# gogojjh/M-LOAM

Hardware: NVIDIA B200
Metric: scan_to_map_lidar_frames_per_sec (higher is better)
Workload: dtype f32/f64

## Files before the change

### m-loam_b200/csrc/api.cu

```cuda
#include <cstdio>
#include <cstdlib>
#include <cstring>
#include <new>

#include "ctx.h"
#include "host_util.h"

using namespace mloam;

namespace mloam {

ProfScope::ProfScope(Ctx *ctx, const char *nm) : c(ctx), name(nm) {
  if (!c->prof_on) return;
  auto get = [&]() {
    cudaEvent_t e;
    if (!c->evt_pool.empty()) {
      e = c->evt_pool.back();
      c->evt_pool.pop_back();
    } else {
      cudaEventCreate(&e);
    }
    return e;
  };
  a = get();
  b = get();
  cudaEventRecord(a, c->stream);
}
ProfScope::~ProfScope() {
  if (!a) return;
  cudaEventRecord(b, c->stream);
  c->pending.push_back(Ctx::PendingEvt{name, a, b});
}
void prof_collect(Ctx *c) {
  for (auto &p : c->pending) {
    float ms = 0.f;
    if (cudaEventSynchronize(p.b) == cudaSuccess && cudaEventElapsedTime(&ms, p.a, p.b) == cudaSuccess) {
      ProfSlot &s = c->prof[p.name];
      s.ms += ms;
      s.launches += 1;
    }
    c->evt_pool.push_back(p.a);
    c->evt_pool.push_back(p.b);
  }
  c->pending.clear();
}

}

extern "C" {

const char *mloam_version(void) { return "mloam_b200 0.1 (sm_100a)"; }

void mloam_default_params(mloam_params_t *p) {
  memset(p, 0, sizeof(*p));
  p->n_scans = 64;
  p->distance_sq_threshold = 25.0f;
  p->nearby_scan = 2.5f;
  p->min_match_sq_dis = 1.0f;
  p->min_plane_dis = 0.2f;
  p->n_neigh = 5;
  p->check_fov = 0;
  p->point_plane_factor = 1;
  p->point_edge_factor = 1;
  p->huber_a = 0.1;
  p->eig_thre = 100.0;
  p->cov_trace = 0.0075;
  p->max_outer = 2;
  p->max_inner = 30;
  p->map_cell = 0.0f;
  p->corner_leaf = 0.2f;
  p->surf_leaf = 0.4f;
  p->gf_method = 0, p->gf_ratio = 1.0f, p->gf_seed = 0;
}

int mloam_ctx_create(int device, const mloam_params_t *params, mloam_ctx_t **out) {
  if (!out) return MLOAM_E_INVALID;
  *out = nullptr;
  int ndev = 0;
  if (cudaGetDeviceCount(&ndev) != cudaSuccess || ndev <= 0 || device < 0 || device >= ndev) return MLOAM_E_NO_DEVICE;
  cudaDeviceProp prop;
  if (cudaGetDeviceProperties(&prop, device) != cudaSuccess) return MLOAM_E_NO_DEVICE;
  if (prop.major != 10) {
    fprintf(stderr, "mloam_b200: device %d is sm_%d%d; this library carries sm_100a code only\n", device, prop.major,
            prop.minor);
    return MLOAM_E_NO_DEVICE;
  }
  if (cudaSetDevice(device) != cudaSuccess) return MLOAM_E_NO_DEVICE;
  mloam_ctx *h = new (std::nothrow) mloam_ctx();
  if (!h) return MLOAM_E_INVALID;
  Ctx *c = &h->c;
  c->device = device;
  c->sm_count = prop.multiProcessorCount;
  if (params) c->params = *params;
  else mloam_default_params(&c->params);
  if (cudaStreamCreateWithFlags(&c->stream, cudaStreamNonBlocking) != cudaSuccess ||
      cudaStreamCreateWithFlags(&c->stream2, cudaStreamNonBlocking) != cudaSuccess ||
      cudaEventCreateWithFlags(&c->ev_fork, cudaEventDisableTiming) != cudaSuccess ||
      cudaEventCreateWithFlags(&c->ev_join, cudaEventDisableTiming) != cudaSuccess ||
      cudaEventCreateWithFlags(&c->ev_maps, cudaEventDisableTiming) != cudaSuccess ||
      cudaStreamCreateWithFlags(&c->stream3, cudaStreamNonBlocking) != cudaSuccess ||
      cudaEventCreateWithFlags(&c->ev_fork3, cudaEventDisableTiming) != cudaSuccess ||
      cudaEventCreateWithFlags(&c->ev_join3, cudaEventDisableTiming) != cudaSuccess ||
      cudaStreamCreateWithFlags(&c->stream4, cudaStreamNonBlocking) != cudaSuccess ||
      cudaStreamCreateWithFlags(&c->stream5, cudaStreamNonBlocking) != cudaSuccess ||
      cudaEventCreateWithFlags(&c->ev_fork4, cudaEventDisableTiming) != cudaSuccess ||
      cudaEventCreateWithFlags(&c->ev_join4, cudaEventDisableTiming) != cudaSuccess ||
      cudaEventCreateWithFlags(&c->ev_fork5, cudaEventDisableTiming) != cudaSuccess ||
      cudaEventCreateWithFlags(&c->ev_join5, cudaEventDisableTiming) != cudaSuccess ||
      cudaEventCreateWithFlags(&c->ev_next, cudaEventDisableTiming) != cudaSuccess ||
      cudaMallocHost(&c->pinned, kPinnedBytes) != cudaSuccess || c->lm_state.reserve(sizeof(LMState) + 64) != cudaSuccess ||
      c->scratch[7].reserve(4096) != cudaSuccess) {
    delete h;
    return MLOAM_E_CUDA;
  }
  c->pinned_cap = kPinnedBytes;
  memset(c->pinned, 0, kPinnedBytes);
  cudaMemset(c->scratch[7].p, 0, 4096);
  if (const char *e = getenv("MLOAM_DISABLE_GRAPHS")) c->use_graphs = (e[0] == '0' || e[0] == '\0') ? 1 : 0;
  if (const char *e = getenv("MLOAM_KNN_TRACE")) c->knn_trace_on = e[0] == '1';
  if (const char *e = getenv("MLOAM_KNN_MB")) {
    const int v = atoi(e);
    if (v >= 2 && v <= 4) c->knn_min_blocks = v;
  }
  if (const char *e = getenv("MLOAM_KNN_TMA_MIN")) c->knn_tma_min = (unsigned)strtoul(e, nullptr, 10);
  if (const char *e = getenv("MLOAM_LOOKAHEAD")) c->use_lookahead = (e[0] == '0') ? 0 : 1;
  if (const char *e = getenv("MLOAM_STAMP")) c->stamp_on = e[0] == '1';
  if (const char *e = getenv("MLOAM_FUSE_ITER")) c->fuse_iter = (e[0] == '0') ? 0 : 1;
  if (const char *e = getenv("MLOAM_DISABLE_SEEDS")) c->use_seeds = (e[0] == '0' || e[0] == '\0') ? 1 : 0;
  *out = h;
  return MLOAM_OK;
}

void mloam_ctx_destroy(mloam_ctx_t *h) {
  if (!h) return;
  Ctx *c = &h->c;
  cudaSetDevice(c->device);
  cudaStreamSynchronize(c->stream);
  mloam_comm_destroy(h);
  for (auto &g : c->graphs)
    if (g.exec) cudaGraphExecDestroy(g.exec);
  c->graphs.clear();
  prof_collect(c);
  for (auto e : c->evt_pool) cudaEventDestroy(e);
  for (auto &m : c->maps) {
    m.sorted.release(), m.orig.release(), m.cells.release(), m.rank_of.release(), m.tile_sums.release(), m.hdr.release();
  }
  for (int i = 0; i < 4; i++) c->scan_pts[i].release(), c->feat_valid[i].release(), c->feat_coeff[i].release(), c->feat_nn[i].release(), c->knn_pos[i].release(), c->knn_changed[i].release(), c->knn_anchor[i].release(), c->knn_heavy[i].release();
  for (int i = 0; i < 2; i++) c->gf_work[i].release();
  c->knn_heavy_list.release(), c->knn_trace.release();
  c->partials.release(), c->lm_state.release();
  for (auto &s : c->scratch) s.release();
  c->frame_main.release(), c->frame_alt.release(), c->next_in.release(), c->stamps.release();
  if (c->pinned) cudaFreeHost(c->pinned);
  if (c->own_stream && c->stream) cudaStreamDestroy(c->stream);
  if (c->stream2) cudaStreamSynchronize(c->stream2), cudaStreamDestroy(c->stream2);
  if (c->ev_fork) cudaEventDestroy(c->ev_fork);
  if (c->ev_join) cudaEventDestroy(c->ev_join);
  if (c->ev_maps) cudaEventDestroy(c->ev_maps);
  if (c->stream3) cudaStreamSynchronize(c->stream3), cudaStreamDestroy(c->stream3);
  if (c->ev_fork3) cudaEventDestroy(c->ev_fork3);
  if (c->ev_join3) cudaEventDestroy(c->ev_join3);
  if (c->stream4) cudaStreamSynchronize(c->stream4), cudaStreamDestroy(c->stream4);
  if (c->stream5) cudaStreamSynchronize(c->stream5), cudaStreamDestroy(c->stream5);
  for (cudaEvent_t ev : {c->ev_fork4, c->ev_join4, c->ev_fork5, c->ev_join5, c->ev_next})
    if (ev) cudaEventDestroy(ev);
  delete h;
}

int mloam_set_params(mloam_ctx_t *h, const mloam_params_t *p) {
  if (!h || !p) return MLOAM_E_INVALID;
  if (p->n_neigh != 5 && p->n_neigh != 10) return fail(&h->c, MLOAM_E_INVALID, "n_neigh must be 5 or 10");
  h->c.params = *p;
  h->c.prefetched.valid = false;
  return MLOAM_OK;
}

int mloam_set_stream(mloam_ctx_t *h, void *s) {
  if (!h) return MLOAM_E_INVALID;
  Ctx *c = &h->c;
  cudaStreamSynchronize(c->stream);
  if (c->own_stream && c->stream) cudaStreamDestroy(c->stream);
  c->stream = (cudaStream_t)s;
  c->own_stream = false;
  return MLOAM_OK;
}

int mloam_sync(mloam_ctx_t *h) {
  if (!h) return MLOAM_E_INVALID;
  MLOAM_CUDA_OK(&h->c, cudaStreamSynchronize(h->c.stream));
  return MLOAM_OK;
}
const char *mloam_last_error(mloam_ctx_t *h) { return h ? h->c.err.c_str() : "null context"; }
long long mloam_launch_count(mloam_ctx_t *h) { return h ? h->c.launches : 0; }

int mloam_profile_enable(mloam_ctx_t *h, int on) {
  if (!h) return MLOAM_E_INVALID;
  h->c.prof_on = on != 0;
  return MLOAM_OK;
}
int mloam_profile_get(mloam_ctx_t *h, const char *name, double *ms_total, long long *launches) {
  if (!h || !name) return MLOAM_E_INVALID;
  Ctx *c = &h->c;
  cudaStreamSynchronize(c->stream);
  prof_collect(c);
  if (!strcmp(name, "graph_capture_failures")) {
    if (ms_total) *ms_total = 0.0;
    if (launches) *launches = c->graph_capture_failures;
    return MLOAM_OK;
  }
  if (!strncmp(name, "knn_slow_rec", 12) && name[12] >= '0' && name[12] <= '9') {
    long long v = 0;
    MLOAM_CUDA_OK(c, cudaMemcpy(&v, c->scratch[7].as<char>() + kKnnPathStatsOffset + 160 + 8 * (size_t)(name[12] - '0'), 8, cudaMemcpyDeviceToHost));
    if (ms_total) *ms_total = 0.0;
    if (launches) *launches = v;
    return MLOAM_OK;
  }
  static const char *kBlind[8] = {"knn_blind_cycles_coarse", "knn_blind_cycles_ring1", "knn_blind_cycles_finish", "knn_blind_ring1_points",
                                  "knn_blind_finish_points", "knn_blind_finish_blocks", "knn_blind_finish_cells", "knn_blind_finish_queries"};
  for (int k = 0; k < 8; k++)
    if (!strcmp(name, kBlind[k])) {
      unsigned long long v = 0;
      MLOAM_CUDA_OK(c, cudaMemcpy(&v, c->scratch[7].as<char>() + kKnnPathStatsOffset + 96 + 8 * (size_t)k, 8, cudaMemcpyDeviceToHost));
      if (ms_total) *ms_total = 0.0;
      if (launches) *launches = (long long)v;
      return MLOAM_OK;
    }
  static const char *kPaths[12] = {"knn_keep_matched", "knn_keep_rejected", "knn_ball", "knn_blind", "knn_max_query_cycles",
                                   "knn_queries_over_32k_cycles", "knn_queries_over_64k_cycles", "knn_cycles_keep_matched",
                                   "knn_cycles_keep_rejected", "knn_cycles_ball", "knn_cycles_blind", "knn_slowest_query"};
  for (int k = 0; k < 12; k++)
    if (!strcmp(name, kPaths[k])) {
      unsigned long long v = 0;
      const size_t off = kKnnPathStatsOffset + (k < 7 ? 4 * (size_t)k : 32 + 8 * (size_t)(k - 7));
      MLOAM_CUDA_OK(c, cudaMemcpy(&v, c->scratch[7].as<char>() + off, k < 7 ? 4 : 8, cudaMemcpyDeviceToHost));
      if (ms_total) *ms_total = 0.0;
      if (launches) *launches = (long long)v;
      return MLOAM_OK;
    }
  auto it = c->prof.find(name);
  if (ms_total) *ms_total = it == c->prof.end() ? 0.0 : it->second.ms;
  if (launches) *launches = it == c->prof.end() ? 0 : it->second.launches;
  return MLOAM_OK;
}
int mloam_profile_reset(mloam_ctx_t *h) {
  if (!h) return MLOAM_E_INVALID;
  cudaStreamSynchronize(h->c.stream);
  prof_collect(&h->c);
  cudaMemset(h->c.scratch[7].as<char>() + kKnnPathStatsOffset, 0, 256);
  h->c.prof.clear();
  return MLOAM_OK;
}

int mloam_map_build_device(mloam_ctx_t *h, int slot, const mloam_point_t *d_pts, int m, float cell) {
  if (!h) return MLOAM_E_INVALID;
  Ctx *c = &h->c;
  cudaSetDevice(c->device);
  return map_build_device(c, slot, reinterpret_cast<const float4 *>(d_pts), m, pick_cell(c, cell));
}

int mloam_map_build(mloam_ctx_t *h, int slot, const mloam_point_t *h_pts, int m, float cell) {
  if (!h || (!h_pts && m > 0) || m < 0) return MLOAM_E_INVALID;
  Ctx *c = &h->c;
  cudaSetDevice(c->device);
  DevBuf &stage = c->scratch[0];
  MLOAM_CUDA_OK(c, stage.reserve(sizeof(float4) * (size_t)(m + 1)));
  MLOAM_CUDA_OK(c, cudaMemcpyAsync(stage.p, h_pts, sizeof(float4) * (size_t)m, cudaMemcpyHostToDevice, c->stream));
  return map_build_device(c, slot, stage.as<float4>(), m, pick_cell(c, cell));
}

__global__ void k_stamp(unsigned long long *slot) {
  unsigned long long t;
  asm volatile("mov.u64 %0, %%globaltimer;" : "=l"(t));
  *slot = t;
}
}
namespace mloam {
void stamp(Ctx *c, const char *label) {
  if (!c->stamp_on || c->stamp_mute || c->stamp_n >= 256) return;
  if (c->stamps.reserve(256 * sizeof(unsigned long long)) != cudaSuccess) return;
  if ((int)c->stamp_labels.size() <= c->stamp_n) c->stamp_labels.resize(c->stamp_n + 1);
  c->stamp_labels[c->stamp_n] = label;
  k_stamp<<<1, 1, 0, c->stream>>>(c->stamps.as<unsigned long long>() + c->stamp_n);
  c->stamp_n++;
}
}
extern "C" {
int mloam_debug_stamps(mloam_ctx_t *h, unsigned long long *out_ns, int cap, int *n) {
  if (!h || !out_ns || !n) return MLOAM_E_INVALID;
  cudaSetDevice(h->c.device);
  *n = h->c.stamp_n < cap ? h->c.stamp_n : cap;
  if (*n <= 0) return MLOAM_OK;
  if (cudaStreamSynchronize(h->c.stream) != cudaSuccess) return MLOAM_E_CUDA;
  return cudaMemcpy(out_ns, h->c.stamps.p, sizeof(unsigned long long) * (size_t)*n, cudaMemcpyDeviceToHost) == cudaSuccess ? MLOAM_OK : MLOAM_E_CUDA;
}
const char *mloam_debug_stamp_label(mloam_ctx_t *h, int i) {
  if (!h || i < 0 || i >= (int)h->c.stamp_labels.size()) return "";
  return h->c.stamp_labels[i].c_str();
}

int mloam_debug_knn_trace(mloam_ctx_t *h, unsigned *out, int n_queries) {
  if (!h || !out || n_queries <= 0 || h->c.knn_trace.cap < 16 * (size_t)n_queries) return MLOAM_E_INVALID;
  cudaSetDevice(h->c.device);
  if (cudaStreamSynchronize(h->c.stream) != cudaSuccess) return MLOAM_E_CUDA;
  return cudaMemcpy(out, h->c.knn_trace.p, 16 * (size_t)n_queries, cudaMemcpyDeviceToHost) == cudaSuccess ? MLOAM_OK : MLOAM_E_CUDA;
}

int mloam_map_size(mloam_ctx_t *h, int slot) {
  if (!h || slot < 0 || slot >= MLOAM_NUM_MAPS || !h->c.maps[slot].built) return -1;
  return h->c.maps[slot].m;
}

int mloam_knn(mloam_ctx_t *h, int slot, const mloam_point_t *h_q, int nq, const double *pose7, int k, float max_sqdist,
              int *h_idx, float *h_sqdist) {
  if (!h || nq < 0 || (nq > 0 && (!h_q || !h_idx || !h_sqdist))) return MLOAM_E_INVALID;
  Ctx *c = &h->c;
  cudaSetDevice(c->device);
  if (nq == 0) return MLOAM_OK;
  MLOAM_CUDA_OK(c, c->scratch[1].reserve(sizeof(float4) * (size_t)nq));
  MLOAM_CUDA_OK(c, c->scratch[2].reserve(sizeof(int) * (size_t)nq * k));
  MLOAM_CUDA_OK(c, c->scratch[3].reserve(sizeof(float) * (size_t)nq * k));
  MLOAM_CUDA_OK(c, cudaMemcpyAsync(c->scratch[1].p, h_q, sizeof(float4) * (size_t)nq, cudaMemcpyHostToDevice, c->stream));
  double *d_pose = nullptr;
  if (pose7) {
    int rc = upload_pose(c, pose7, &d_pose);
    if (rc) return rc;
  }
  int rc = knn_device(c, slot, c->scratch[1].as<float4>(), nq, d_pose, k, max_sqdist, c->scratch[2].as<int>(),
                      c->scratch[3].as<float>());
  if (rc) return rc;
  MLOAM_CUDA_OK(c, cudaMemcpyAsync(h_idx, c->scratch[2].p, sizeof(int) * (size_t)nq * k, cudaMemcpyDeviceToHost, c->stream));
  MLOAM_CUDA_OK(c, cudaMemcpyAsync(h_sqdist, c->scratch[3].p, sizeof(float) * (size_t)nq * k, cudaMemcpyDeviceToHost, c->stream));
  MLOAM_CUDA_OK(c, cudaStreamSynchronize(c->stream));
  return MLOAM_OK;
}

int mloam_match_from_map(mloam_ctx_t *h, int slot, int type, const mloam_point_t *h_pts, int n, const double *pose7,
                         unsigned char *h_valid, double *h_coeffs, int *h_nn) {
  if (!h || n < 0 || !pose7 || (n > 0 && (!h_pts || !h_valid || !h_coeffs))) return MLOAM_E_INVALID;
  Ctx *c = &h->c;
  cudaSetDevice(c->device);
  if (n == 0) return MLOAM_OK;
  const int t = type == 's' ? 1 : 0;
  const int K = c->params.n_neigh;
  MLOAM_CUDA_OK(c, c->scan_pts[t].reserve(sizeof(float4) * (size_t)n));
  int rc = reserve_feat(c, t, n);
  if (rc) return rc;
  MLOAM_CUDA_OK(c, cudaMemcpyAsync(c->scan_pts[t].p, h_pts, sizeof(float4) * (size_t)n, cudaMemcpyHostToDevice, c->stream));
  double *d_pose;
  rc = upload_pose(c, pose7, &d_pose);
  if (rc) return rc;
  rc = match_from_map_device(c, slot, type, c->scan_pts[t].as<float4>(), n, nullptr, d_pose, match_cfg(c),
                             c->feat_valid[t].as<unsigned char>(), c->feat_coeff[t].as<float>(), c->feat_nn[t].as<int>());
  if (rc) return rc;
  std::vector<float> cf((size_t)n * 6);
  MLOAM_CUDA_OK(c, cudaMemcpyAsync(h_valid, c->feat_valid[t].p, (size_t)n, cudaMemcpyDeviceToHost, c->stream));
  MLOAM_CUDA_OK(c, cudaMemcpyAsync(cf.data(), c->feat_coeff[t].p, sizeof(float) * 6 * (size_t)n, cudaMemcpyDeviceToHost, c->stream));
  if (h_nn)
    MLOAM_CUDA_OK(c, cudaMemcpyAsync(h_nn, c->feat_nn[t].p, sizeof(int) * (size_t)K * n, cudaMemcpyDeviceToHost, c->stream));
  MLOAM_CUDA_OK(c, cudaStreamSynchronize(c->stream));
  for (size_t i = 0; i < (size_t)n * 6; i++) h_coeffs[i] = (double)cf[i];
  return MLOAM_OK;
}

int mloam_factor_evaluate(mloam_ctx_t *h, int kind, int n, const double *h_points, const double *h_coeffs,
                          const double *h_sqrt_info, const double *h_params, double *h_residuals, double *h_jacobians) {
  if (!h || n < 0 || kind < 0 || kind > 4 || (n > 0 && (!h_points || !h_coeffs || !h_params || !h_residuals)))
    return MLOAM_E_INVALID;
  Ctx *c = &h->c;
  cudaSetDevice(c->device);
  if (n == 0) return MLOAM_OK;
  const int rows = kind == 2 ? 3 : 1;
  const int cols = kind >= 3 ? 21 : 7;
  const int np = kind >= 3 ? 21 : 7;
  DevBuf &dp = c->scratch[1], &dc = c->scratch[2], &ds = c->scratch[3], &dr = c->scratch[4], &dj = c->scratch[5], &dx = c->scratch[6];
  MLOAM_CUDA_OK(c, dp.reserve(sizeof(double) * 3 * (size_t)n));
  MLOAM_CUDA_OK(c, dc.reserve(sizeof(double) * 6 * (size_t)n));
  MLOAM_CUDA_OK(c, ds.reserve(sizeof(double) * (size_t)n));
  MLOAM_CUDA_OK(c, dr.reserve(sizeof(double) * rows * (size_t)n));
  MLOAM_CUDA_OK(c, dj.reserve(sizeof(double) * rows * cols * (size_t)n));
  MLOAM_CUDA_OK(c, dx.reserve(sizeof(double) * 32));
  cudaStream_t st = c->stream;
  MLOAM_CUDA_OK(c, cudaMemcpyAsync(dp.p, h_points, sizeof(double) * 3 * (size_t)n, cudaMemcpyHostToDevice, st));
  MLOAM_CUDA_OK(c, cudaMemcpyAsync(dc.p, h_coeffs, sizeof(double) * 6 * (size_t)n, cudaMemcpyHostToDevice, st));
  if (h_sqrt_info) MLOAM_CUDA_OK(c, cudaMemcpyAsync(ds.p, h_sqrt_info, sizeof(double) * (size_t)n, cudaMemcpyHostToDevice, st));
  MLOAM_CUDA_OK(c, cudaMemcpyAsync(dx.p, h_params, sizeof(double) * np, cudaMemcpyHostToDevice, st));
  int rc = factor_evaluate_device(c, kind, n, dp.as<double>(), dc.as<double>(), h_sqrt_info ? ds.as<double>() : nullptr,
                                  dx.as<double>(), dr.as<double>(), h_jacobians ? dj.as<double>() : nullptr);
  if (rc) return rc;
  MLOAM_CUDA_OK(c, cudaMemcpyAsync(h_residuals, dr.p, sizeof(double) * rows * (size_t)n, cudaMemcpyDeviceToHost, st));
  if (h_jacobians)
    MLOAM_CUDA_OK(c, cudaMemcpyAsync(h_jacobians, dj.p, sizeof(double) * rows * cols * (size_t)n, cudaMemcpyDeviceToHost, st));
  MLOAM_CUDA_OK(c, cudaStreamSynchronize(st));
  return MLOAM_OK;
}

int mloam_normal_equations(mloam_ctx_t *h, int n, const unsigned char *h_types, const double *h_points, const double *h_coeffs,
                           double sqrt_info, double huber_a, const double *pose7, double *H36, double *g6, double *cost) {
  if (!h || n < 0 || !pose7 || !H36 || !g6 || !cost || (n > 0 && (!h_types || !h_points || !h_coeffs))) return MLOAM_E_INVALID;
  Ctx *c = &h->c;
  cudaSetDevice(c->device);
  std::vector<float4> pts[2];
  std::vector<float> cf[2];
  for (int i = 0; i < n; i++) {
    const int t = h_types[i] == 's' ? 1 : 0;
    pts[t].push_back(make_float4((float)h_points[i * 3], (float)h_points[i * 3 + 1], (float)h_points[i * 3 + 2], 0.f));
    for (int k = 0; k < 6; k++) cf[t].push_back((float)h_coeffs[(size_t)i * 6 + k]);
  }
  FeatSet sets[2];
  for (int t = 0; t < 2; t++) {
    const int nt = (int)pts[t].size();
    MLOAM_CUDA_OK(c, c->scan_pts[t].reserve(sizeof(float4) * (size_t)(nt + 1)));
    int rc = reserve_feat(c, t, nt);
    if (rc) return rc;
    if (nt > 0) {
      MLOAM_CUDA_OK(c, cudaMemcpyAsync(c->scan_pts[t].p, pts[t].data(), sizeof(float4) * nt, cudaMemcpyHostToDevice, c->stream));
      MLOAM_CUDA_OK(c, cudaMemcpyAsync(c->feat_coeff[t].p, cf[t].data(), sizeof(float) * 6 * nt, cudaMemcpyHostToDevice, c->stream));
      MLOAM_CUDA_OK(c, cudaMemsetAsync(c->feat_valid[t].p, 1, nt, c->stream));
    }
    sets[t] = FeatSet{c->scan_pts[t].as<float4>(), c->feat_valid[t].as<unsigned char>(), c->feat_coeff[t].as<float>(), nt, t, nullptr};
  }
  double *d_pose;
  int rc = upload_pose(c, pose7, &d_pose);
  if (rc) return rc;
  MLOAM_CUDA_OK(c, c->scratch[6].reserve(sizeof(double) * 32));
  rc = linearize_device(c, sets, 2, sqrt_info, huber_a, d_pose, 0, 0, c->scratch[6].as<double>());
  if (rc) return rc;
  double *ne = reinterpret_cast<double *>(c->pinned) + 64;
  MLOAM_CUDA_OK(c, cudaMemcpyAsync(ne, c->scratch[6].p, sizeof(double) * 30, cudaMemcpyDeviceToHost, c->stream));
  MLOAM_CUDA_OK(c, cudaStreamSynchronize(c->stream));
  int q = 0;
  for (int i = 0; i < 6; i++)
    for (int j = i; j < 6; j++) H36[i * 6 + j] = H36[j * 6 + i] = ne[q++];
  for (int k = 0; k < 6; k++) g6[k] = ne[21 + k];
  *cost = ne[27];
  return MLOAM_OK;
}

__global__ void k_pose_plus(const double *x, const double *d, const double *V, double *out) {
  if (threadIdx.x == 0) mloam::pose_plus(x, d, V, out);
}
int mloam_pose_plus(mloam_ctx_t *h, const double *x7, const double *delta6, const double *V36, double *out7) {
  if (!h || !x7 || !delta6 || !out7) return MLOAM_E_INVALID;
  Ctx *c = &h->c;
  cudaSetDevice(c->device);
  double *stage = reinterpret_cast<double *>(c->pinned) + 128;
  for (int k = 0; k < 7; k++) stage[k] = x7[k];
  for (int k = 0; k < 6; k++) stage[8 + k] = delta6[k];
  for (int k = 0; k < 36; k++) stage[16 + k] = V36 ? V36[k] : (k % 7 == 0 ? 1.0 : 0.0);
  MLOAM_CUDA_OK(c, c->scratch[6].reserve(sizeof(double) * 64));
  double *d = c->scratch[6].as<double>();
  MLOAM_CUDA_OK(c, cudaMemcpyAsync(d, stage, sizeof(double) * 52, cudaMemcpyHostToDevice, c->stream));
  k_pose_plus<<<1, 32, 0, c->stream>>>(d, d + 8, d + 16, d + 56);
  c->launches++;
  MLOAM_CUDA_OK(c, cudaMemcpyAsync(stage + 56, d + 56, sizeof(double) * 7, cudaMemcpyDeviceToHost, c->stream));
  MLOAM_CUDA_OK(c, cudaStreamSynchronize(c->stream));
  for (int k = 0; k < 7; k++) out7[k] = stage[56 + k];
  return MLOAM_OK;
}

}
```

### m-loam_b200/csrc/common.cuh

```cuda
#pragma once
#include <cuda_runtime.h>
#include <stdint.h>
#include <math.h>

#define MLOAM_FULL_MASK 0xffffffffu

namespace mloam {

struct D3 {
  double x, y, z;
};
__host__ __device__ inline D3 operator+(const D3 &a, const D3 &b) { return {a.x + b.x, a.y + b.y, a.z + b.z}; }
__host__ __device__ inline D3 operator-(const D3 &a, const D3 &b) { return {a.x - b.x, a.y - b.y, a.z - b.z}; }
__host__ __device__ inline D3 operator*(double s, const D3 &a) { return {s * a.x, s * a.y, s * a.z}; }
__host__ __device__ inline D3 neg(const D3 &a) { return {-a.x, -a.y, -a.z}; }
__host__ __device__ inline double dot(const D3 &a, const D3 &b) { return a.x * b.x + a.y * b.y + a.z * b.z; }
__host__ __device__ inline D3 cross(const D3 &a, const D3 &b) {
  return {a.y * b.z - a.z * b.y, a.z * b.x - a.x * b.z, a.x * b.y - a.y * b.x};
}
__host__ __device__ inline double norm(const D3 &a) { return sqrt(dot(a, a)); }

struct M33 {
  double m[9];
};
__host__ __device__ inline D3 matvec(const M33 &A, const D3 &v) {
  return {A.m[0] * v.x + A.m[1] * v.y + A.m[2] * v.z, A.m[3] * v.x + A.m[4] * v.y + A.m[5] * v.z,
          A.m[6] * v.x + A.m[7] * v.y + A.m[8] * v.z};
}
__host__ __device__ inline D3 vecmat(const D3 &v, const M33 &A) {
  return {v.x * A.m[0] + v.y * A.m[3] + v.z * A.m[6], v.x * A.m[1] + v.y * A.m[4] + v.z * A.m[7],
          v.x * A.m[2] + v.y * A.m[5] + v.z * A.m[8]};
}
__host__ __device__ inline D3 vecmatT(const D3 &v, const M33 &A) { return matvec(A, v); }
__host__ __device__ inline D3 vec_skew(const D3 &v, const D3 &p) {
  return {v.y * p.z - v.z * p.y, -v.x * p.z + v.z * p.x, v.x * p.y - v.y * p.x};
}

struct Q4 {
  double x, y, z, w;
};
__host__ __device__ inline Q4 qmul(const Q4 &a, const Q4 &b) {
  return {a.w * b.x + a.x * b.w + a.y * b.z - a.z * b.y, a.w * b.y + a.y * b.w + a.z * b.x - a.x * b.z,
          a.w * b.z + a.z * b.w + a.x * b.y - a.y * b.x, a.w * b.w - a.x * b.x - a.y * b.y - a.z * b.z};
}
__host__ __device__ inline Q4 qconj(const Q4 &q) { return {-q.x, -q.y, -q.z, q.w}; }
__host__ __device__ inline Q4 qnormalized(const Q4 &q) {
  double n = sqrt(q.x * q.x + q.y * q.y + q.z * q.z + q.w * q.w);
  return {q.x / n, q.y / n, q.z / n, q.w / n};
}
__host__ __device__ inline D3 qrot(const Q4 &q, const D3 &v) {
  D3 u{q.x, q.y, q.z};
  D3 uv = cross(u, v);
  uv = uv + uv;
  return v + q.w * uv + cross(u, uv);
}
__host__ __device__ inline M33 qmat(const Q4 &q) {
  const double tx = 2 * q.x, ty = 2 * q.y, tz = 2 * q.z;
  const double twx = tx * q.w, twy = ty * q.w, twz = tz * q.w;
  const double txx = tx * q.x, txy = ty * q.x, txz = tz * q.x;
  const double tyy = ty * q.y, tyz = tz * q.y, tzz = tz * q.z;
  return M33{{1 - (tyy + tzz), txy - twz, txz + twy, txy + twz, 1 - (txx + tzz), tyz - twx, txz - twy, tyz + twx,
              1 - (txx + tyy)}};
}

struct PoseD {
  Q4 q;
  D3 t;
};
__host__ __device__ inline PoseD pose_from_param(const double *x) {
  return PoseD{Q4{x[3], x[4], x[5], x[6]}, D3{x[0], x[1], x[2]}};
}
__host__ __device__ inline float3 associate(const PoseD &T, float px, float py, float pz) {
  D3 v = qrot(T.q, D3{(double)px, (double)py, (double)pz}) + T.t;
  return make_float3((float)v.x, (float)v.y, (float)v.z);
}

__host__ __device__ inline void pose_plus(const double *x, const double *delta, const double *V, double *out) {
  double dx[6];
  for (int i = 0; i < 6; i++) {
    double s = 0;
    for (int j = 0; j < 6; j++) s += V[i * 6 + j] * delta[j];
    dx[i] = s;
  }
  out[0] = x[0] + dx[0], out[1] = x[1] + dx[1], out[2] = x[2] + dx[2];
  const Q4 dq{dx[3] / 2.0, dx[4] / 2.0, dx[5] / 2.0, 1.0};
  const Q4 qn = qnormalized(qmul(Q4{x[3], x[4], x[5], x[6]}, dq));
  out[3] = qn.x, out[4] = qn.y, out[5] = qn.z, out[6] = qn.w;
}


struct GridHdr {
  int ox, oy, oz;
  int nx, ny, nz;
  int n_cells;
  int level;
  float cell, inv_cell;
  int n_sorted;
  int n_occupied;
  int bb_min[3], bb_max[3];
  int ticket;
  int pad[1];
};

struct MapView {
  const float4 *sorted;
  const float4 *orig;
  const unsigned *cell_start;
  const GridHdr *hdr;
  int m;
};

struct GridP {
  int ox, oy, oz, nx, ny, nz;
  float cell, inv_cell;
};
__device__ __forceinline__ GridP load_grid(const MapView &mv) {
  GridP g;
  if (!mv.hdr) {
    g.ox = g.oy = g.oz = 0, g.nx = g.ny = g.nz = 0, g.cell = 1.0f, g.inv_cell = 1.0f;
    return g;
  }
  const int4 a = __ldg(reinterpret_cast<const int4 *>(mv.hdr));
  const int4 b = __ldg(reinterpret_cast<const int4 *>(mv.hdr) + 1);
  const float2 c = __ldg(reinterpret_cast<const float2 *>(mv.hdr) + 4);
  g.ox = a.x, g.oy = a.y, g.oz = a.z, g.nx = a.w, g.ny = b.x, g.nz = b.y, g.cell = c.x, g.inv_cell = c.y;
  return g;
}
static_assert(sizeof(GridHdr) % 16 == 0, "GridHdr is read with vector loads");

#define MLOAM_P2P_MAX_RANKS 8
#define MLOAM_P2P_BYTES 8192
struct P2PView {
  double *slots[MLOAM_P2P_MAX_RANKS];
  unsigned *flags[MLOAM_P2P_MAX_RANKS];
  unsigned long long *epoch;
  int nranks, rank;
};

#define MLOAM_NE_MAX 92

struct LMState {
  double x[7];
  double xc[7];
  double H[36];
  double g[6];
  double cost;
  double scale[6];
  double diag[6];
  double radius, decrease_factor;
  double model_cost_change;
  double x_norm;
  double V_update[36];
  double eig[6];
  double H0[36];
  double initial_cost;
  int is_degenerate;
  int reuse_diagonal;
  int iteration;
  int num_invalid;
  int done;
  int termination;
  int total_iterations;
  int rows;
  int n_valid[2];
  int max_inner;
  int pad;
  int work[2];
  int min_corr;
  int skipped;
  long long dbg_cycles[4];
};

}
```

### m-loam_b200/csrc/ctx.h

```cpp
#pragma once
#include <cuda_runtime.h>
#include <map>
#include <string>
#include <vector>

#include "../../include/mloam_b200.h"
#include "common.cuh"

namespace mloam {

inline unsigned long long &alloc_epoch() {
  static unsigned long long e = 0;
  return e;
}

struct FitSet {
  const float4 *sorted;
  const float4 *pts;
  int n;
  const int *d_n;
  const int *pos;
  unsigned char *valid;
  float *coeff;
  int *nn;
  int is_plane;
  const unsigned char *changed;
};
struct PendingFit {
  FitSet set[2];
  int K = 0;
  float min_plane_dis = 0.f;
  int check_fov = 0;
};

struct DevBuf {
  void *p = nullptr;
  size_t cap = 0;
  cudaError_t reserve(size_t bytes) {
    if (bytes <= cap) return cudaSuccess;
    size_t want = bytes + bytes / 4 + 256;
    if (p) cudaFree(p);
    p = nullptr;
    cap = 0;
    alloc_epoch()++;
    cudaError_t e = cudaMalloc(&p, want);
    if (e == cudaSuccess) cap = want;
    return e;
  }
  void release() {
    if (p) cudaFree(p);
    p = nullptr;
    cap = 0;
  }
  template <typename T>
  T *as() const {
    return reinterpret_cast<T *>(p);
  }
};

#define MLOAM_MAX_RINGS 1024
#define MLOAM_MAX_LIDARS 16

constexpr size_t kMapStatsOffset = 16384;

struct MapStorage {
  DevBuf sorted, orig, cells, rank_of, tile_sums, hdr;
  unsigned capacity = 0;
  int m = 0;
  float cell = 0.f;
  float auto_cell = 0.25f;
  bool built = false;
  MapView view() const {
    MapView v;
    v.sorted = sorted.as<float4>();
    v.orig = orig.as<float4>();
    v.cell_start = cells.as<unsigned>();
    v.hdr = hdr.as<GridHdr>();
    v.m = m;
    return v;
  }
  float auto_cell_pick(const void *pinned, int slot) {
    if (built && pinned) {
      const GridHdr *h = reinterpret_cast<const GridHdr *>(reinterpret_cast<const char *>(pinned) + kMapStatsOffset + 64 * slot);
      if (h->n_occupied > 0 && h->n_sorted > 0 && h->cell > 0.f) {
        const float avg = (float)h->n_sorted / (float)h->n_occupied;
        float cur = h->cell;
        if (avg < 2.5f && cur < 1.0f) cur *= 2.0f;
        else if (avg > 40.0f && cur > 0.125f) cur *= 0.5f;
        auto_cell = cur;
      }
    }
    return auto_cell;
  }
};

constexpr size_t kPinnedScanInfo = 32768, kPinnedScanInfoNext = 40960;
constexpr size_t kKnnPathStatsOffset = 3072;

struct ProfSlot {
  double ms = 0;
  long long launches = 0;
};

struct MatchCfg {
  float min_match_sq_dis, min_plane_dis;
  int n_neigh, check_fov;
};

struct Ctx {
  int device = 0;
  int sm_count = 148;
  cudaStream_t stream = nullptr;
  bool own_stream = true;
  cudaStream_t stream2 = nullptr;
  cudaEvent_t ev_fork = nullptr, ev_join = nullptr;
  cudaStream_t stream3 = nullptr;
  cudaEvent_t ev_fork3 = nullptr, ev_join3 = nullptr;
  cudaEvent_t ev_maps = nullptr;
  bool maps_pending = false;
  mloam_params_t params;
  std::string err;
  long long launches = 0;

  MapStorage maps[MLOAM_NUM_MAPS];

  DevBuf scan_pts[4];
  DevBuf feat_valid[4];
  DevBuf feat_coeff[4];
  DevBuf feat_nn[4];
  DevBuf knn_pos[4];
  DevBuf knn_changed[4];
  DevBuf knn_anchor[4];
  DevBuf gf_work[2];
  DevBuf knn_heavy[4];
  DevBuf knn_heavy_list;
  int knn_rot = 0;
  int knn_parity = 0;
  DevBuf partials;
  DevBuf lm_state;
  void *ticket_zeroed_for = nullptr;
  DevBuf scratch[10];
  void *pinned = nullptr;
  size_t pinned_cap = 0;

  bool prof_on = false;
  std::map<std::string, ProfSlot> prof;
  struct PendingEvt {
    std::string name;
    cudaEvent_t a, b;
  };
  std::vector<PendingEvt> pending;
  std::vector<cudaEvent_t> evt_pool;

  void *d_ring_stage = nullptr;
  int *d_ring_cnt = nullptr;
  int *d_extract_status = nullptr;
  struct ScanRef {
    const float4 *surf;
    int n_surf;
    const int *d_n_surf;
    const float4 *corner;
    int n_corner;
    const int *d_n_corner;
    const double *sinfo_surf, *sinfo_corner;
  };
  struct Features {
    bool valid = false;
    bool host = false;
    const void *key_ptr = nullptr;
    int n = 0, n_scans = 0, parity = 0;
    ScanRef S{};
  };
  struct NextSweep {
    bool set = false, host = false;
    const void *key_ptr = nullptr;
    const float4 *d_cloud = nullptr;
    const int *d_scan_start = nullptr, *d_scan_end = nullptr;
    int n = 0, n_scans = 0;
  };
  Features prefetched;
  NextSweep next;
  const void *cloud_key = nullptr;
  const int *next_host_ss = nullptr, *next_host_se = nullptr;
  bool next_pending = false;
  int frame_parity = 0;
  int use_lookahead = 1;
  bool stamp_mute = false;
  DevBuf frame_main, frame_alt, next_in;
  cudaStream_t stream4 = nullptr, stream5 = nullptr;
  cudaEvent_t ev_fork4 = nullptr, ev_join4 = nullptr, ev_fork5 = nullptr, ev_join5 = nullptr, ev_next = nullptr;
  struct GraphEntry {
    unsigned long long key = 0, epoch = 0;
    cudaGraphExec_t exec = nullptr;
    int launches = 0, seen = 0, s2m_ran = 0;
    ScanRef S{};
    Features prefetched_out{};
  };
  std::vector<GraphEntry> graphs;
  bool smem_opt_in_gf = false;
  bool smem_opt_in[3] = {false, false, false};
  long long graph_capture_failures = 0;
  int use_graphs = 1;
  unsigned knn_tma_min = 8;
  DevBuf knn_trace;
  bool knn_trace_on = false;
  bool stamp_on = false;
  DevBuf stamps;
  int stamp_n = 0;
  std::vector<std::string> stamp_labels;
  int knn_min_blocks = 4;
  int use_seeds = 1;
  int s2m_ran = 0;
  int lm_min_corr = 0;
  double lm_eig_thre = -1.0;
  int fuse_iter = 1;
  PendingFit pending_fit;
  bool lin_two_pass = false;
  int want_eig = 1;
  bool lidar_merge = false;
  int n_lidars = 1;
  double lidar_ext[MLOAM_MAX_LIDARS][7];
  bool has_ext = false;
  double ext[7] = {0, 0, 0, 0, 0, 0, 1};
  void *nccl_comm = nullptr;
  int nranks = 1, rank = 0;
  void *p2p_local = nullptr;
  void *p2p_peer[MLOAM_P2P_MAX_RANKS] = {nullptr};
  void *p2p_view = nullptr;
  bool p2p_on = false;
  bool p2p_collective = false;
};

struct ProfScope {
  Ctx *c;
  cudaEvent_t a = nullptr, b = nullptr;
  const char *name;
  ProfScope(Ctx *ctx, const char *nm);
  ~ProfScope();
};
void prof_collect(Ctx *c);

#define MLOAM_CUDA_OK(ctx, expr)                                                                      \
  do {                                                                                                \
    cudaError_t _e = (expr);                                                                          \
    if (_e != cudaSuccess) {                                                                          \
      (ctx)->err = std::string(#expr) + ": " + cudaGetErrorString(_e);                                \
      return MLOAM_E_CUDA;                                                                            \
    }                                                                                                 \
  } while (0)

int map_build_device(Ctx *c, int slot, const float4 *d_pts, int m, float cell);
int knn_device(Ctx *c, int slot, const float4 *d_q, int nq, const double *d_pose7_or_null, int k, float max_sqdist,
               int *d_idx, float *d_sqd);
int match_from_map_device(Ctx *c, int slot, int type, const float4 *d_pts, int n, const int *d_n, const double *d_pose7,
                          const MatchCfg &cfg, unsigned char *d_valid, float *d_coeff, int *d_nn, int *d_work = nullptr);

struct MatchJob {
  int slot;
  int type;
  const float4 *pts;
  int n;
  const int *d_n;
  unsigned char *valid;
  float *coeff;
  int *nn;
  int seeded;
};
int match_pair_device(Ctx *c, const MatchJob *jobs, int n_jobs, const double *d_pose7, const MatchCfg &cfg, int *d_work, int buf_base = 0,
                      bool defer_fit = false);

int match_from_scan_device(Ctx *c, int slot, int type, const float4 *d_pts, int n, const double *d_pose7, unsigned char *d_valid,
                           float *d_coeff, int *d_nn3);
int track_cloud_device(Ctx *c, const float4 *d_prev_less_sharp, int n_pls, const float4 *d_prev_less_flat, int n_plf,
                       const float4 *d_cur_sharp, int n_cs, const float4 *d_cur_flat, int n_cf, const double *pose_ini7,
                       double *pose_out7, mloam_solve_stats_t *stats);

struct FeatSet {
  const float4 *pts;
  const unsigned char *valid;
  const float *coeff;
  int n;
  int is_plane;
  const int *d_n;
  const double *sinfo;
  const unsigned char *mask;
};
int linearize_device(Ctx *c, const FeatSet *sets, int n_sets, double sqrt_info, double huber_a, const double *d_pose7,
                     int use_state, int lm_mode, double *d_out29);
int lm_init_state(Ctx *c, const double *pose7_host, int max_inner, double eig_thre);
void eig_report_host(const double *H36, double *w6);
int factor_evaluate_device(Ctx *c, int kind, int n, const double *d_points, const double *d_coeffs, const double *d_sqrt_info,
                           const double *d_params, double *d_res, double *d_jac);

int transform_points_device(Ctx *c, float4 *d_pts, int n, const int *d_n, const double *d_pose7);

int gf_select_set_device(Ctx *c, int t, const FeatSet &fs, const double *d_pose7, double default_sinfo, int method, double gf_ratio,
                         unsigned long long seed, unsigned char **d_mask_out);

int sqrt_info_device(Ctx *c, const float *d_cov6, int n, double *d_sinfo);

int comm_allreduce_doubles(Ctx *c, double *d_buf, int count);

struct ExtractOut {
  float4 *sharp, *less_sharp, *flat, *less_flat;
  int *counts;
};
int extract_device(Ctx *c, const float4 *d_cloud, int n, const int *d_scan_start, const int *d_scan_end, int n_scans,
                   ExtractOut out, float *d_curv_or_null, int *d_label_or_null);
void stamp(Ctx *c, const char *label);
int project_cloud_device(Ctx *c, const float4 *d_in, int n, int vertical_scans, int horizon_scans, double roi_range, float4 *d_out,
                         int *d_scan_start, int *d_scan_end, int *d_n_out);
int transform_segments_device(Ctx *c, float4 *d_pts, int n, const int *d_off, int n_seg, const float *d_mat12);
int voxel_downsample_cov_device(Ctx *c, const float4 *d_in, const float *d_cov6, const float *d_trace, int n, const int *d_n_in, float leaf,
                                float trace_threshold, float4 *d_out, float *d_cov6_out, float *d_trace_out, int *d_n_out, int work_slot = 5);
void scan_exclusive(Ctx *c, const int *d_in, int *d_out, int n, int *d_tmp, int *d_total);
int merge_lidars_device(Ctx *c, ExtractOut out, int n_cap_less, int n_cap_lflat, int n_lidars, int rings_per_lidar, const float *d_ext12,
                        int *d_off);
int voxel_downsample_device(Ctx *c, const float4 *d_in, int n, const int *d_n_in, float leaf, int intensity_last, float4 *d_out,
                            int *d_n_out, int work_slot = 5);

}

struct mloam_ctx {
  mloam::Ctx c;
};
```

### m-loam_b200/csrc/match_kernels.cu

```cuda
#include <cstdlib>

#include "ctx.h"
#include "fit.cuh"
#include "knn.cuh"
#include "match_fit.cuh"

namespace mloam {

constexpr int MWARPS = 8;

struct KnnSet {
  MapView map;
  const float4 *pts;
  int n;
  const int *d_n;
  int *pos;
  int seeded;
  unsigned char *changed;
  float4 *anchor;
  const unsigned char *heavy_in;
  unsigned char *heavy_out;
};

struct HeavyQ {
  const int *list_in;
  const int *cnt_in;
  int *list_out;
  int *cnt_out;
  int *cnt_zero;
};

template <int K, int MB>
__global__ void __launch_bounds__(MWARPS * 32, MB)
    k_match_knn(KnnSet a, KnnSet b, const double *__restrict__ pose7, float min_match_sq_dis, HeavyQ hq,
                unsigned *__restrict__ path_stats, unsigned tma_min, unsigned *__restrict__ trace) {
  __shared__ KnnSmem ksm[MWARPS];
  const int lane = threadIdx.x & 31;
  KnnSmem &ks = ksm[threadIdx.x >> 5];
  unsigned long long t_enter = 0ull;
  if (trace) asm volatile("mov.u64 %0, %%globaltimer;" : "=l"(t_enter));
  knn_smem_init(ks, lane, tma_min);
  __shared__ GridP s_grid[2];
  __shared__ PoseD s_pose;
  if (threadIdx.x == 0) s_grid[0] = load_grid(a.map), s_grid[1] = load_grid(b.map), s_pose = pose_from_param(pose7);
  __syncthreads();
  const int na = a.d_n ? min(a.n, *a.d_n) : a.n;
  const int nb = b.d_n ? min(b.n, *b.d_n) : b.n;
  const int n = na + nb;
  const int gw = blockIdx.x * MWARPS + (threadIdx.x >> 5), n_warps = gridDim.x * MWARPS;
  if (hq.cnt_zero && gw == 0 && lane == 0) *hq.cnt_zero = 0;
  const bool listed = hq.list_in != nullptr;
  const int n_heavy = listed ? min(__ldg(hq.cnt_in), n) : 0;
  const int it_a = n_heavy > gw ? (n_heavy - gw + n_warps - 1) / n_warps : 0;
  const int it_b = n > gw ? (n - gw + n_warps - 1) / n_warps : 0;
#pragma unroll 1
  for (int it = 0; it < it_a + it_b; it++) {
    int i;
    if (it < it_a) {
      i = __ldg(hq.list_in + gw + it * n_warps);
    } else {
      i = gw + (it - it_a) * n_warps;
      if (listed) {
        const unsigned char *hin = i < na ? a.heavy_in : b.heavy_in;
        if (hin && hin[i < na ? i : i - na]) continue;
      }
    }
    const float4 p = __ldg(i < na ? a.pts + i : b.pts + (i - na));
    const bool in_a = i < na;
    const int j = in_a ? i : i - na;
    const long long t_query = (path_stats || trace) ? clock64() : 0ll;
    int path = 3;
    const float3 sel = associate(s_pose, p.x, p.y, p.z);
    const GridP &g = s_grid[in_a ? 0 : 1];
    Best best;
    int *const pos_out = (in_a ? a.pos : b.pos) + (size_t)j * K;
    const int seeded = in_a ? a.seeded : b.seeded;
    unsigned char *const changed = in_a ? a.changed : b.changed;
    float4 *const anchor = (in_a ? a.anchor : b.anchor) + j;
    int prev = -1, newpos = -1;
    bool done = false;
    float r2 = 3.0e38f;
    if (seeded) {
      if (lane < K) prev = pos_out[lane];
      const float4 an = *anchor;
      const float mx = sel.x - an.x, my = sel.y - an.y, mz = sel.z - an.z;
      const float moved = sqrtf(mx * mx + my * my + mz * mz);
      const bool within = an.w > 0.0f && moved + 2e-5f < an.w;
      if (__shfl_sync(MLOAM_FULL_MASK, prev, 0) < 0) {
        if (within) {
          done = true;
          path = 1;
        }
      } else {
        unsigned long long key = MLOAM_KEY_NONE;
        unsigned d2b = 0u;
        if (lane < K) {
          const float4 v = __ldg((in_a ? a.map.sorted : b.map.sorted) + prev);
          const float ex = v.x - sel.x, ey = v.y - sel.y, ez = v.z - sel.z;
          d2b = __float_as_uint(ex * ex + ey * ey + ez * ez);
          key = ((unsigned long long)d2b << 32) | (unsigned)__float_as_int(v.w);
        }
        r2 = __uint_as_float(__reduce_max_sync(MLOAM_FULL_MASK, d2b));
        if (within) {
          int rank = 0;
#pragma unroll
          for (int k = 0; k < K; k++) {
            const unsigned long long other = __shfl_sync(MLOAM_FULL_MASK, key, k);
            if (other < key) rank++;
          }
#pragma unroll
          for (int k = 0; k < K; k++) {
            const int rk = __shfl_sync(MLOAM_FULL_MASK, rank, k), pk = __shfl_sync(MLOAM_FULL_MASK, prev, k);
            if (rk == lane) newpos = pk;
          }
          if (!(r2 < min_match_sq_dis)) {
            newpos = -1;
            if (lane == 0) *anchor = make_float4(sel.x, sel.y, sel.z, 0.0f);
          }
          done = true;
          path = 0;
        }
      }
    }
    if (!done) {
      float explored = 0.0f;
      bool found = false;
      if (r2 < min_match_sq_dis)
        found = warp_knn_seeded<K, K + 1>(in_a ? a.map : b.map, g, ks, sel.x, sel.y, sel.z, r2, 0.1f * g.cell,
                                             lane, best, &explored);
      if (!found) {
        KnnDbg dbg = {0, 0, 0, 0, 0, 0};
        const long long t_blind = (path_stats || trace) ? clock64() : 0ll;
        warp_knn<K, true, K + 1>(in_a ? a.map : b.map, g, ks, sel.x, sel.y, sel.z, min_match_sq_dis, lane, best, &explored, 0.05f,
                                 (path_stats || trace) ? &dbg : nullptr);
        if (trace && lane == 0) {
          unsigned *tr = trace + 4 * (size_t)((in_a ? 0 : na) + j);
          tr[1] = (unsigned)dbg.t_ring1, tr[2] = (unsigned)dbg.t_ball, tr[3] = ((unsigned)dbg.ring1_pts << 20) | ((unsigned)(dbg.ball_pts & 0xfff) << 8) | (unsigned)(dbg.ball_steps & 0xff);
        }
        if (path_stats && lane == 0) {
          unsigned long long *q = reinterpret_cast<unsigned long long *>(path_stats + 24);
          atomicAdd(q + 0, 0ull), atomicAdd(q + 1, (unsigned long long)dbg.t_ring1);
          atomicAdd(q + 2, (unsigned long long)dbg.t_ball), atomicAdd(q + 3, (unsigned long long)dbg.ring1_pts);
          atomicAdd(q + 4, (unsigned long long)dbg.ball_pts), atomicAdd(q + 5, (unsigned long long)dbg.ball_steps);
          atomicAdd(q + 6, (unsigned long long)dbg.ball_rows), atomicAdd(q + 7, dbg.t_ball ? 1ull : 0ull);
          const long long dt_blind = clock64() - t_blind;
          if (dt_blind > 90000) {
            long long *rec = reinterpret_cast<long long *>(path_stats + 40);
            rec[0] = dt_blind, rec[1] = 0, rec[2] = dbg.t_ring1, rec[3] = dbg.t_ball, rec[4] = dbg.ring1_pts;
            rec[5] = dbg.ball_pts, rec[6] = dbg.ball_rows, rec[7] = dbg.ball_steps, rec[8] = (in_a ? 0 : 1) * 1000000 + j;
            rec[9] = (long long)(t_blind - t_query);
          }
        }
      }
      path = found ? 2 : 3;
      const unsigned long long kK = best_key(best, K - 1), kK1 = best_key(best, K);
      const bool ok = kK != MLOAM_KEY_NONE && key_d2(kK) < min_match_sq_dis;
      newpos = (ok && lane < K) ? best.pos : -1;
      float slack = 0.0f;
      if (ok) {
        const float rK = sqrtf(key_d2(kK));
        float lb = explored;
        if (kK1 != MLOAM_KEY_NONE) lb = fminf(lb, sqrtf(key_d2(kK1)));
        slack = 0.5f * (lb - rK) - 2e-5f;
      } else {
        float lbK = explored;
        if (kK != MLOAM_KEY_NONE) lbK = fminf(lbK, sqrtf(key_d2(kK)));
        slack = lbK - sqrtf(min_match_sq_dis) - 2e-5f;
      }
      if (lane == 0) *anchor = make_float4(sel.x, sel.y, sel.z, slack);
    }
    if (lane < K) pos_out[lane] = newpos;
    if (changed) {
      const bool diff = __any_sync(MLOAM_FULL_MASK, lane < K && (!seeded || newpos != prev));
      if (lane == 0) changed[j] = diff ? 1 : 0;
    }
    if (path_stats && lane == 0) {
      const unsigned long long dt = (unsigned long long)(clock64() - t_query);
      atomicAdd(path_stats + path, 1u);
      atomicAdd(reinterpret_cast<unsigned long long *>(path_stats + 8) + path, dt);
      atomicMax(path_stats + 4, (unsigned)(dt > 0xffffffffull ? 0xffffffffull : dt));
      if (dt > 32768ull) atomicAdd(path_stats + 5, 1u);
      if (dt > 65536ull) atomicAdd(path_stats + 6, 1u);
      atomicMax(reinterpret_cast<unsigned long long *>(path_stats + 16),
                (dt << 32) | ((unsigned long long)path << 30) | ((unsigned long long)(in_a ? 0 : 1) << 29) | (unsigned)(j & 0x1fffffff));
    }
    if (trace && lane == 0) trace[4 * (size_t)((in_a ? 0 : na) + j)] = (unsigned)(clock64() - t_query) | ((unsigned)path << 30);
    unsigned char *const hout = in_a ? a.heavy_out : b.heavy_out;
    if (hout && lane == 0) {
      hout[j] = path >= 2 ? 1 : 0;
      if (path >= 2 && hq.list_out) hq.list_out[atomicAdd(hq.cnt_out, 1)] = i;
    }
  }
  if (trace && lane == 0) {
    unsigned long long t_exit;
    asm volatile("mov.u64 %0, %%globaltimer;" : "=l"(t_exit));
    unsigned long long *w = reinterpret_cast<unsigned long long *>(trace + 4 * (size_t)(a.n + b.n + 1)) + 2 * (size_t)(blockIdx.x * MWARPS + (threadIdx.x >> 5));
    w[0] = t_enter, w[1] = t_exit;
  }
}

template <int K>
__global__ void __launch_bounds__(128) k_match_fit(FitSet a, FitSet b, const double *__restrict__ pose7, float min_plane_dis, int check_fov) {
  const int na = a.d_n ? min(a.n, *a.d_n) : a.n;
  const int nb = b.d_n ? min(b.n, *b.d_n) : b.n;
  const PoseD T = pose_from_param(pose7);
  for (int i = blockIdx.x * blockDim.x + threadIdx.x; i < na + nb; i += gridDim.x * blockDim.x) {
    if (i < na) fit_one<K>(a, i, T, min_plane_dis, check_fov);
    else fit_one<K>(b, i - na, T, min_plane_dis, check_fov);
  }
}

int match_pair_device(Ctx *c, const MatchJob *jobs, int n_jobs, const double *d_pose7, const MatchCfg &cfg, int *d_work, int buf_base, bool defer_fit) {
  (void)d_work;
  if (n_jobs < 1 || n_jobs > 2 || (buf_base != 0 && buf_base != 2)) {
    c->err = "match: 1 or 2 jobs";
    return MLOAM_E_INVALID;
  }
  if (cfg.n_neigh != 5 && cfg.n_neigh != 10) {
    c->err = "match_from_map: n_neigh must be 5 or 10";
    return MLOAM_E_INVALID;
  }
  const int K = cfg.n_neigh;
  KnnSet ks[2];
  FitSet fs[2];
  int n_upper = 0;
  bool flip = false;
  for (int t = 0; t < 2; t++) {
    KnnSet &k = ks[t];
    FitSet &f = fs[t];
    memset(&k, 0, sizeof(k));
    memset(&f, 0, sizeof(f));
    if (t >= n_jobs || jobs[t].n <= 0) continue;
    const MatchJob &J = jobs[t];
    if (J.slot < 0 || J.slot >= MLOAM_NUM_MAPS || !c->maps[J.slot].built) {
      c->err = "match_from_map: map slot not built";
      return MLOAM_E_STATE;
    }
    if (J.type != 'c' && J.type != 's') {
      c->err = "match_from_map: type must be 'c' or 's'";
      return MLOAM_E_INVALID;
    }
    DevBuf &pb = c->knn_pos[buf_base + t];
    MLOAM_CUDA_OK(c, pb.reserve(sizeof(int) * (size_t)K * (size_t)(J.n + 1)));
    k.map = c->maps[J.slot].view();
    DevBuf &cb = c->knn_changed[buf_base + t];
    MLOAM_CUDA_OK(c, cb.reserve((size_t)(J.n + 1)));
    k.pts = J.pts, k.n = J.n, k.d_n = J.d_n, k.pos = pb.as<int>();
    DevBuf &ab = c->knn_anchor[buf_base + t];
    MLOAM_CUDA_OK(c, ab.reserve(sizeof(float4) * (size_t)(J.n + 1)));
    k.seeded = J.seeded, k.changed = cb.as<unsigned char>(), k.anchor = ab.as<float4>();
    DevBuf &hb = c->knn_heavy[buf_base + t];
    const size_t half = ((size_t)J.n + 256) & ~(size_t)255;
    MLOAM_CUDA_OK(c, hb.reserve(2 * half));
    k.heavy_in = J.seeded ? hb.as<unsigned char>() + half * (size_t)c->knn_parity : nullptr;
    k.heavy_out = hb.as<unsigned char>() + half * (size_t)(J.seeded ? (c->knn_parity ^ 1) : c->knn_parity);
    flip = flip || J.seeded;
    f.changed = (J.seeded && !J.nn) ? cb.as<unsigned char>() : nullptr;
    f.sorted = k.map.sorted, f.pts = J.pts, f.n = J.n, f.d_n = J.d_n, f.pos = pb.as<int>();
    f.valid = J.valid, f.coeff = J.coeff, f.nn = J.nn, f.is_plane = J.type == 's' ? 1 : 0;
    n_upper += J.n;
  }
  if (n_upper <= 0) return MLOAM_OK;
  HeavyQ hq{nullptr, nullptr, nullptr, nullptr, nullptr};
  {
    DevBuf &hl = c->knn_heavy_list;
    const size_t ints = 2 * ((size_t)n_upper + 64) + 16;
    if (hl.cap < sizeof(int) * ints) {
      MLOAM_CUDA_OK(c, hl.reserve(sizeof(int) * ints));
      MLOAM_CUDA_OK(c, cudaMemsetAsync(hl.p, 0, hl.cap, c->stream));
    }
    int *cnt = hl.as<int>();
    int *lists = hl.as<int>() + 16;
    const size_t half_l = (size_t)n_upper + 64;
    if (!flip) {
      c->knn_rot = 0;
      MLOAM_CUDA_OK(c, cudaMemsetAsync(cnt, 0, 3 * sizeof(int), c->stream));
    }
    const int k = c->knn_rot;
    if (flip) hq.list_in = lists + half_l * (size_t)(k & 1), hq.cnt_in = cnt + k % 3;
    hq.list_out = lists + half_l * (size_t)((k + 1) & 1), hq.cnt_out = cnt + (k + 1) % 3, hq.cnt_zero = cnt + (k + 2) % 3;
    c->knn_rot = k + 1;
  }
  if (flip) c->knn_parity ^= 1;
  cudaStream_t st = c->stream;
  {
    ProfScope ps(c, "match");
    unsigned *path_stats = (c->prof_on && !getenv("MLOAM_KNN_NO_STATS")) ? reinterpret_cast<unsigned *>(c->scratch[7].as<char>() + kKnnPathStatsOffset) : nullptr;
    unsigned *trace = nullptr;
    if (c->knn_trace_on) {
      MLOAM_CUDA_OK(c, c->knn_trace.reserve(16 * (size_t)(n_upper + 1) + 16 * 8 * 4 * 148 + 64));
      MLOAM_CUDA_OK(c, cudaMemsetAsync(c->knn_trace.p, 0, 16 * (size_t)(n_upper + 1) + 16 * 8 * 4 * 148, st));
      trace = c->knn_trace.as<unsigned>();
    }
    const int mb = c->knn_min_blocks;
    int nb = (n_upper + MWARPS - 1) / MWARPS;
    if (nb > mb * c->sm_count) nb = mb * c->sm_count;
#define MLOAM_LAUNCH_KNN(KK, MBB) \
  k_match_knn<KK, MBB><<<nb, MWARPS * 32, 0, st>>>(ks[0], ks[1], d_pose7, cfg.min_match_sq_dis, hq, path_stats, c->knn_tma_min, trace)
    if (K == 5) {
      if (mb == 2) MLOAM_LAUNCH_KNN(5, 2);
      else if (mb == 3) MLOAM_LAUNCH_KNN(5, 3);
      else MLOAM_LAUNCH_KNN(5, 4);
    } else {
      if (mb == 2) MLOAM_LAUNCH_KNN(10, 2);
      else if (mb == 3) MLOAM_LAUNCH_KNN(10, 3);
      else MLOAM_LAUNCH_KNN(10, 4);
    }
#undef MLOAM_LAUNCH_KNN
    c->launches++;
  }
  c->pending_fit.K = 0;
  if (defer_fit && !fs[0].nn && !fs[1].nn) {
    c->pending_fit.set[0] = fs[0], c->pending_fit.set[1] = fs[1];
    c->pending_fit.K = K, c->pending_fit.min_plane_dis = cfg.min_plane_dis, c->pending_fit.check_fov = cfg.check_fov;
  } else {
    ProfScope ps(c, "fit");
    int nb = (n_upper + 127) / 128;
    if (nb > 4 * c->sm_count) nb = 4 * c->sm_count;
    if (K == 5) k_match_fit<5><<<nb, 128, 0, st>>>(fs[0], fs[1], d_pose7, cfg.min_plane_dis, cfg.check_fov);
    else k_match_fit<10><<<nb, 128, 0, st>>>(fs[0], fs[1], d_pose7, cfg.min_plane_dis, cfg.check_fov);
    c->launches++;
  }
  MLOAM_CUDA_OK(c, cudaGetLastError());
  return MLOAM_OK;
}

int match_from_map_device(Ctx *c, int slot, int type, const float4 *d_pts, int n, const int *d_n, const double *d_pose7,
                          const MatchCfg &cfg, unsigned char *d_valid, float *d_coeff, int *d_nn, int *d_work) {
  MatchJob j{slot, type, d_pts, n, d_n, d_valid, d_coeff, d_nn, 0};
  return match_pair_device(c, &j, 1, d_pose7, cfg, d_work);
}

}
```

### m-loam_b200/csrc/pipeline.cu

```cuda
#include <cstdio>
#include <cstring>

#include "ctx.h"
#include "host_util.h"

using namespace mloam;

namespace {

typedef Ctx::ScanRef ScanRef;

int scan2map_enqueue(Ctx *c, const ScanRef &S, const double *pose_init7) {
  const mloam_params_t &P = c->params;
  c->s2m_ran = 0;
  const MapStorage &MS = c->maps[MLOAM_MAP_SURF], &MC = c->maps[MLOAM_MAP_CORNER];
  if (!MS.built || !MC.built) return fail(c, MLOAM_E_STATE, "scan2map: build MLOAM_MAP_SURF and MLOAM_MAP_CORNER first");
  if (!((MS.m > 50) && (MC.m > 10))) return MLOAM_OK;
  c->s2m_ran = 1;
  struct CollectiveScope {
    Ctx *c;
    explicit CollectiveScope(Ctx *cc) : c(cc) { c->p2p_collective = true; }
    ~CollectiveScope() { c->p2p_collective = false; }
  } collective_scope(c);
  int rc = reserve_feat(c, 0, S.n_corner);
  if (rc) return rc;
  rc = reserve_feat(c, 1, S.n_surf);
  if (rc) return rc;
  rc = lm_init_state(c, pose_init7, P.max_inner, P.eig_thre);
  if (rc) return rc;
  LMState *st = c->lm_state.as<LMState>();
  const double *d_pose = st->x;
  const double sinfo = map_sqrt_info(P.cov_trace);
  const MatchCfg cfg = match_cfg(c);
  int *h_done = reinterpret_cast<int *>(reinterpret_cast<char *>(c->pinned) + 2048);
  const int nc_use = P.point_edge_factor ? S.n_corner : 0, ns_use = P.point_plane_factor ? S.n_surf : 0;
  FeatSet sets[2] = {
      FeatSet{S.corner, c->feat_valid[0].as<unsigned char>(), c->feat_coeff[0].as<float>(), nc_use, 0, S.d_n_corner, S.sinfo_corner},
      FeatSet{S.surf, c->feat_valid[1].as<unsigned char>(), c->feat_coeff[1].as<float>(), ns_use, 1, S.d_n_surf, S.sinfo_surf}};
  for (int outer = 0; outer < P.max_outer; outer++) {
    {
      const int seeded = (outer > 0 && c->use_seeds) ? 1 : 0;
      MatchJob jobs[2] = {
          MatchJob{MLOAM_MAP_CORNER, 'c', S.corner, nc_use, S.d_n_corner, c->feat_valid[0].as<unsigned char>(),
                   c->feat_coeff[0].as<float>(), nullptr, seeded},
          MatchJob{MLOAM_MAP_SURF, 's', S.surf, ns_use, S.d_n_surf, c->feat_valid[1].as<unsigned char>(),
                   c->feat_coeff[1].as<float>(), nullptr, seeded}};
      const bool defer_fit = c->fuse_iter && P.gf_method == 0;
      rc = match_pair_device(c, jobs, 2, d_pose, cfg, &st->work[0], 0, defer_fit);
      if (rc) return rc;
      stamp(c, "match");
    }
    sets[0].mask = sets[1].mask = nullptr;
    if (P.gf_method != 0) {
      const bool fork_gf = !c->prof_on && sets[0].n > 0 && sets[1].n > 0;
      if (fork_gf) {
        MLOAM_CUDA_OK(c, cudaEventRecord(c->ev_fork3, c->stream));
        MLOAM_CUDA_OK(c, cudaStreamWaitEvent(c->stream3, c->ev_fork3, 0));
      }
      for (int t = 0; t < 2; t++) {
        if (sets[t].n <= 0) continue;
        unsigned char *mask = nullptr;
        cudaStream_t main_stream = c->stream;
        if (fork_gf && t == 0) c->stream = c->stream3;
        rc = gf_select_set_device(c, t, sets[t], d_pose, sinfo, P.gf_method, (double)P.gf_ratio,
                                  (unsigned long long)P.gf_seed + 2ull * (unsigned long long)outer + (unsigned long long)t, &mask);
        c->stream = main_stream;
        if (rc) return rc;
        if (fork_gf && t == 0) MLOAM_CUDA_OK(c, cudaEventRecord(c->ev_join3, c->stream3));
        sets[t].mask = mask;
      }
      if (fork_gf) MLOAM_CUDA_OK(c, cudaStreamWaitEvent(c->stream, c->ev_join3, 0));
    }
    if (P.gf_method != 0) stamp(c, "gf");
    c->want_eig = 0;
    c->lin_two_pass = c->fuse_iter && P.max_inner == 1;
    rc = linearize_device(c, sets, 2, sinfo, P.huber_a, nullptr, 1, 1, nullptr);
    c->want_eig = 1;
    const bool second_done = c->lin_two_pass;
    c->lin_two_pass = false;
    if (rc) return rc;
    stamp(c, second_done ? "linearize x2" : "linearize");
    for (int it = 0; it < P.max_inner && !second_done; it++) {
      rc = linearize_device(c, sets, 2, sinfo, P.huber_a, nullptr, 2, 2, nullptr);
      if (rc) return rc;
      stamp(c, "linearize (candidate)");
      if (P.max_inner > 1) {
        MLOAM_CUDA_OK(c, cudaMemcpyAsync(h_done, &st->done, sizeof(int), cudaMemcpyDeviceToHost, c->stream));
        MLOAM_CUDA_OK(c, cudaStreamSynchronize(c->stream));
        if (*h_done) break;
      }
    }
  }
  char *pin = reinterpret_cast<char *>(c->pinned);
  LMState *hs = reinterpret_cast<LMState *>(pin + 4096);
  int *h_cnt = reinterpret_cast<int *>(pin + 3072);
  MLOAM_CUDA_OK(c, cudaMemcpyAsync(hs, st, sizeof(LMState), cudaMemcpyDeviceToHost, c->stream));
  if (S.d_n_surf) MLOAM_CUDA_OK(c, cudaMemcpyAsync(h_cnt, S.d_n_surf, sizeof(int), cudaMemcpyDeviceToHost, c->stream));
  if (S.d_n_corner) MLOAM_CUDA_OK(c, cudaMemcpyAsync(h_cnt + 1, S.d_n_corner, sizeof(int), cudaMemcpyDeviceToHost, c->stream));
  return MLOAM_OK;
}

int scan2map_finish(Ctx *c, const ScanRef &S, const double *pose_init7, double *pose_out7, mloam_solve_stats_t *stats) {
  if (stats) memset(stats, 0, sizeof(*stats));
  for (int k = 0; k < 7; k++) pose_out7[k] = pose_init7[k];
  if (!c->s2m_ran) return MLOAM_OK;
  char *pin = reinterpret_cast<char *>(c->pinned);
  const LMState *hs = reinterpret_cast<const LMState *>(pin + 4096);
  int *h_cnt = reinterpret_cast<int *>(pin + 3072);
  MLOAM_CUDA_OK(c, cudaStreamSynchronize(c->stream));
  if (!S.d_n_surf) h_cnt[0] = S.n_surf;
  if (!S.d_n_corner) h_cnt[1] = S.n_corner;
  for (int k = 0; k < 7; k++) pose_out7[k] = hs->x[k];
  if (hs->termination == 9) {
    for (int k = 0; k < 7; k++) pose_out7[k] = pose_init7[k];
    if (stats) stats->ran = 1, stats->termination = 9;
    return fail(c, MLOAM_E_NCCL, "scan2map: peer-memory exchange failed (a rank did not arrive or the ranks lost lock-step); "
                                  "call mloam_comm_p2p_reset on every rank behind a barrier");
  }
  if (hs->termination == 8) {
    for (int k = 0; k < 7; k++) pose_out7[k] = pose_init7[k];
    if (stats) stats->ran = 1, stats->termination = 8;
    return fail(c, MLOAM_E_STATE, "scan2map: the two-evaluation launch timed out at its grid barrier (GPU shared with a kernel that never "
                                   "yields?); set MLOAM_FUSE_ITER=0 to use one launch per evaluation");
  }
  if (c->prof_on) {
    int khz = 0;
    cudaDeviceGetAttribute(&khz, cudaDevAttrClockRate, c->device);
    if (khz > 0) {
      c->prof["lm_tail_reduce"].ms += (double)hs->dbg_cycles[0] / khz, c->prof["lm_tail_reduce"].launches += hs->dbg_cycles[2];
      c->prof["lm_tail_advance"].ms += (double)hs->dbg_cycles[1] / khz, c->prof["lm_tail_advance"].launches += hs->dbg_cycles[2];
    }
  }
  if (stats) {
    stats->ran = 1;
    stats->n_corner = hs->n_valid[0], stats->n_surf = hs->n_valid[1];
    stats->lm_iterations = hs->total_iterations;
    stats->degenerate = hs->is_degenerate;
    stats->termination = hs->termination;
    stats->final_cost = hs->cost;
    memcpy(stats->eig, hs->eig, sizeof(stats->eig));
    memcpy(stats->H, hs->H0, sizeof(stats->H));
    const double thre = c->lm_eig_thre >= 0.0 ? c->lm_eig_thre : c->params.eig_thre;
    if (!hs->is_degenerate && !hs->skipped && hs->rows > 0 && thre > 0.0) eig_report_host(hs->H0, stats->eig);
    stats->n_surf_in = h_cnt[0], stats->n_corner_in = h_cnt[1];
  }
  return MLOAM_OK;
}

int scan2map_run(Ctx *c, const ScanRef &S, const double *pose_init7, double *pose_out7, mloam_solve_stats_t *stats) {
  int rc = scan2map_enqueue(c, S, pose_init7);
  if (rc) return rc;
  return scan2map_finish(c, S, pose_init7, pose_out7, stats);
}

struct FrameBufs {
  ExtractOut ex;
  float4 *corner_ds, *surf_ds;
  int *n_corner_ds, *n_surf_ds;
};
int frame_bufs(Ctx *c, int n, FrameBufs *F, int parity = 0) {
  DevBuf &B = parity ? c->frame_alt : c->frame_main;
  size_t off = 0;
  auto take = [&](size_t bytes) {
    size_t o = off;
    off += (bytes + 255) & ~(size_t)255;
    return o;
  };
  const size_t N1 = (size_t)n + 16;
  const size_t o_sharp = take(16 * N1), o_less = take(16 * N1), o_flat = take(16 * N1), o_lflat = take(16 * N1);
  const size_t o_cds = take(16 * N1), o_sds = take(16 * N1), o_cnt = take(64);
  MLOAM_CUDA_OK(c, B.reserve(off));
  char *p = B.as<char>();
  F->ex.sharp = reinterpret_cast<float4 *>(p + o_sharp), F->ex.less_sharp = reinterpret_cast<float4 *>(p + o_less);
  F->ex.flat = reinterpret_cast<float4 *>(p + o_flat), F->ex.less_flat = reinterpret_cast<float4 *>(p + o_lflat);
  F->corner_ds = reinterpret_cast<float4 *>(p + o_cds), F->surf_ds = reinterpret_cast<float4 *>(p + o_sds);
  int *cnt = reinterpret_cast<int *>(p + o_cnt);
  F->ex.counts = cnt;
  F->n_corner_ds = cnt + 4, F->n_surf_ds = cnt + 5;
  return MLOAM_OK;
}

bool frame_has_prefetched(const Ctx *c, const void *key_ptr, int n, int n_scans) {
  const Ctx::Features &f = c->prefetched;
  return f.valid && c->use_lookahead && !c->prof_on && f.key_ptr == key_ptr && f.n == n && f.n_scans == n_scans;
}

int features_enqueue(Ctx *c, const float4 *d_cloud, int n, const int *d_scan_start, const int *d_scan_end, int n_scans, int parity,
                     cudaStream_t side, cudaEvent_t ev_fork_v, cudaEvent_t ev_join_v, ScanRef *S_out) {
  const mloam_params_t &P = c->params;
  FrameBufs F;
  int rc = frame_bufs(c, n, &F, parity);
  if (rc) return rc;
  rc = extract_device(c, d_cloud, n, d_scan_start, d_scan_end, n_scans, F.ex, nullptr, nullptr);
  if (rc) return rc;
  stamp(c, "extract");
  const int less_cap = n < 120 * n_scans ? n : 120 * n_scans;
  if (c->n_lidars > 1 || c->lidar_merge) {
    if (n_scans % c->n_lidars != 0) return fail(c, MLOAM_E_INVALID, "frame: n_scans must be n_lidars x rings per LiDAR");
    float *stage = reinterpret_cast<float *>(reinterpret_cast<char *>(c->pinned) + 12288);
    for (int l = 0; l < c->n_lidars; l++) {
      const double *e = c->lidar_ext[l];
      const M33 R = qmat(qnormalized(Q4{e[3], e[4], e[5], e[6]}));
      for (int r = 0; r < 3; r++) {
        for (int k = 0; k < 3; k++) stage[12 * l + 4 * r + k] = (float)R.m[3 * r + k];
        stage[12 * l + 4 * r + 3] = (float)e[r];
      }
    }
    float *d_ext12 = reinterpret_cast<float *>(c->scratch[7].as<char>() + 1024);
    int *d_off = reinterpret_cast<int *>(c->scratch[7].as<char>() + 2048);
    MLOAM_CUDA_OK(c, cudaMemcpyAsync(d_ext12, stage, sizeof(float) * 12 * c->n_lidars, cudaMemcpyHostToDevice, c->stream));
    rc = merge_lidars_device(c, F.ex, less_cap, n, c->n_lidars, n_scans / c->n_lidars, d_ext12, d_off);
    if (rc) return rc;
  } else if (c->has_ext) {
    double *stage = reinterpret_cast<double *>(c->pinned) + 32;
    for (int k = 0; k < 7; k++) stage[k] = c->ext[k];
    double *d_ext = c->scratch[7].as<double>() + 32;
    MLOAM_CUDA_OK(c, cudaMemcpyAsync(d_ext, stage, 7 * sizeof(double), cudaMemcpyHostToDevice, c->stream));
    rc = transform_points_device(c, F.ex.less_sharp, less_cap, F.ex.counts + 1, d_ext);
    if (rc) return rc;
    rc = transform_points_device(c, F.ex.less_flat, n, F.ex.counts + 3, d_ext);
    if (rc) return rc;
  }
  const bool fork_voxel = !c->prof_on;
  if (fork_voxel) {
    MLOAM_CUDA_OK(c, cudaEventRecord(ev_fork_v, c->stream));
    MLOAM_CUDA_OK(c, cudaStreamWaitEvent(side, ev_fork_v, 0));
    cudaStream_t main_stream = c->stream;
    c->stream = side;
    rc = voxel_downsample_device(c, F.ex.less_sharp, less_cap, F.ex.counts + 1, P.corner_leaf, 1, F.corner_ds, F.n_corner_ds, 8);
    c->stream = main_stream;
    if (rc) return rc;
    MLOAM_CUDA_OK(c, cudaEventRecord(ev_join_v, side));
  } else {
    rc = voxel_downsample_device(c, F.ex.less_sharp, less_cap, F.ex.counts + 1, P.corner_leaf, 1, F.corner_ds, F.n_corner_ds, 8);
    if (rc) return rc;
  }
  rc = voxel_downsample_device(c, F.ex.less_flat, n, F.ex.counts + 3, P.surf_leaf, 1, F.surf_ds, F.n_surf_ds, 9);
  if (rc) return rc;
  if (fork_voxel) MLOAM_CUDA_OK(c, cudaStreamWaitEvent(c->stream, ev_join_v, 0));
  stamp(c, "voxel (surf; corner on the side stream)");
  ScanRef S{F.surf_ds, n, F.n_surf_ds, F.corner_ds, less_cap, F.n_corner_ds};
  *S_out = S;
  return MLOAM_OK;
}

int frame_enqueue(Ctx *c, const float4 *d_cloud, int n, const int *d_scan_start, const int *d_scan_end, int n_scans,
                  const float4 *d_surf_map, int n_surf_map, const float4 *d_corner_map, int n_corner_map, int rebuild_maps,
                  const double *pose_init7, ScanRef *S_out) {
  int rc;
  bool forked = false;
  if (rebuild_maps) {
    forked = !c->prof_on;
    if (!forked) {
      if (c->maps_pending) MLOAM_CUDA_OK(c, cudaStreamWaitEvent(c->stream, c->ev_maps, 0));
      rc = map_build_device(c, MLOAM_MAP_SURF, d_surf_map, n_surf_map, pick_cell(c, 0.f));
      if (rc == MLOAM_OK) rc = map_build_device(c, MLOAM_MAP_CORNER, d_corner_map, n_corner_map, pick_cell(c, 0.f));
      if (rc) return rc;
    }
  }
  if (forked) {
    MLOAM_CUDA_OK(c, cudaEventRecord(c->ev_fork, c->stream));
    MLOAM_CUDA_OK(c, cudaStreamWaitEvent(c->stream2, c->ev_fork, 0));
    if (c->maps_pending) {
      cudaStreamCaptureStatus cs = cudaStreamCaptureStatusNone;
      MLOAM_CUDA_OK(c, cudaStreamIsCapturing(c->stream2, &cs));
      if (cs == cudaStreamCaptureStatusActive) MLOAM_CUDA_OK(c, cudaStreamWaitEvent(c->stream2, c->ev_maps, cudaEventWaitExternal));
    }
    cudaStream_t main_stream = c->stream;
    c->stream = c->stream2;
    rc = map_build_device(c, MLOAM_MAP_SURF, d_surf_map, n_surf_map, pick_cell(c, 0.f));
    if (rc == MLOAM_OK) rc = map_build_device(c, MLOAM_MAP_CORNER, d_corner_map, n_corner_map, pick_cell(c, 0.f));
    c->stream = main_stream;
    if (rc) return rc;
    MLOAM_CUDA_OK(c, cudaEventRecord(c->ev_join, c->stream2));
  }
  c->stamp_n = 0;
  stamp(c, "start");
  ScanRef S{};
  int parity = c->frame_parity;
  const void *key_now = c->cloud_key ? c->cloud_key : static_cast<const void *>(d_cloud);
  const bool have = frame_has_prefetched(c, key_now, n, n_scans);
  if (have) {
    S = c->prefetched.S, parity = c->prefetched.parity;
  } else {
    rc = features_enqueue(c, d_cloud, n, d_scan_start, d_scan_end, n_scans, parity, c->stream3, c->ev_fork3, c->ev_join3, &S);
    if (rc) return rc;
  }
  c->prefetched.valid = false;
  c->frame_parity = parity ^ 1;
  bool ahead = false;
  Ctx::Features nf{};
  if (c->next.set && c->use_lookahead && !c->prof_on) {
    const Ctx::NextSweep nx = c->next;
    MLOAM_CUDA_OK(c, cudaEventRecord(c->ev_fork4, c->stream));
    MLOAM_CUDA_OK(c, cudaStreamWaitEvent(c->stream4, c->ev_fork4, 0));
    if (c->next_pending) {
      cudaStreamCaptureStatus cs = cudaStreamCaptureStatusNone;
      MLOAM_CUDA_OK(c, cudaStreamIsCapturing(c->stream4, &cs));
      if (cs == cudaStreamCaptureStatusActive) MLOAM_CUDA_OK(c, cudaStreamWaitEvent(c->stream4, c->ev_next, cudaEventWaitExternal));
    }
    cudaStream_t main_stream = c->stream;
    c->stream = c->stream4;
    c->stamp_mute = true;
    ScanRef Sn{};
    rc = features_enqueue(c, nx.d_cloud, nx.n, nx.d_scan_start, nx.d_scan_end, nx.n_scans, parity ^ 1, c->stream5, c->ev_fork5, c->ev_join5, &Sn);
    c->stamp_mute = false;
    c->stream = main_stream;
    if (rc) return rc;
    MLOAM_CUDA_OK(c, cudaEventRecord(c->ev_join4, c->stream4));
    ahead = true;
    nf.valid = true, nf.host = nx.host, nf.key_ptr = nx.key_ptr, nf.n = nx.n, nf.n_scans = nx.n_scans, nf.parity = parity ^ 1, nf.S = Sn;
  }
  c->next.set = false;
  stamp(c, have ? "features (prefetched)" : "extract + voxel");
  if (forked) MLOAM_CUDA_OK(c, cudaStreamWaitEvent(c->stream, c->ev_join, 0));
  if (forked) stamp(c, "map build join");
  *S_out = S;
  rc = scan2map_enqueue(c, S, pose_init7);
  if (rc) return rc;
  if (ahead) {
    MLOAM_CUDA_OK(c, cudaStreamWaitEvent(c->stream, c->ev_join4, 0));
    stamp(c, "look-ahead join");
    c->prefetched = nf;
  }
  return MLOAM_OK;
}

int stage_next_sweep(Ctx *c) {
  if (!c->next.set || !c->next.host || !c->use_lookahead || c->prof_on) return MLOAM_OK;
  const int n = c->next.n, ns = c->next.n_scans;
  DevBuf &in = c->next_in;
  MLOAM_CUDA_OK(c, in.reserve(sizeof(float4) * (size_t)n + 1024 + 8 * (size_t)ns));
  float4 *d_cloud = in.as<float4>();
  int *d_ss = reinterpret_cast<int *>(in.as<char>() + sizeof(float4) * (size_t)n + 256);
  int *d_se = d_ss + ns;
  int *pin = reinterpret_cast<int *>(reinterpret_cast<char *>(c->pinned) + kPinnedScanInfoNext);
  std::memcpy(pin, c->next_host_ss, sizeof(int) * ns), std::memcpy(pin + MLOAM_MAX_RINGS, c->next_host_se, sizeof(int) * ns);
  MLOAM_CUDA_OK(c, cudaMemcpyAsync(d_ss, pin, sizeof(int) * ns, cudaMemcpyHostToDevice, c->stream4));
  MLOAM_CUDA_OK(c, cudaMemcpyAsync(d_se, pin + MLOAM_MAX_RINGS, sizeof(int) * ns, cudaMemcpyHostToDevice, c->stream4));
  MLOAM_CUDA_OK(c, cudaMemcpyAsync(d_cloud, c->next.key_ptr, sizeof(float4) * (size_t)n, cudaMemcpyHostToDevice, c->stream4));
  MLOAM_CUDA_OK(c, cudaEventRecord(c->ev_next, c->stream4));
  c->next.d_cloud = d_cloud, c->next.d_scan_start = d_ss, c->next.d_scan_end = d_se;
  c->next_pending = true;
  return MLOAM_OK;
}

unsigned long long fnv1a(unsigned long long h, const void *p, size_t n) {
  const unsigned char *b = static_cast<const unsigned char *>(p);
  for (size_t i = 0; i < n; i++) h = (h ^ b[i]) * 1099511628211ull;
  return h;
}

int frame_run(Ctx *c, const float4 *d_cloud, int n, const int *d_scan_start, const int *d_scan_end, int n_scans,
              const float4 *d_surf_map, int n_surf_map, const float4 *d_corner_map, int n_corner_map, int rebuild_maps,
              const double *pose_init7, double *pose_out7, mloam_solve_stats_t *stats) {
  ScanRef S{};
  const bool can_graph = c->use_graphs && c->params.max_inner == 1 && !c->prof_on && (!c->nccl_comm || c->p2p_on);
  if (can_graph) {
    unsigned long long key = 1469598103934665603ull;
    const void *ptrs[5] = {d_cloud, d_scan_start, d_scan_end, d_surf_map, d_corner_map};
    const int ints[7] = {n, n_scans, n_surf_map, n_corner_map, rebuild_maps, c->has_ext ? 1 : 0, c->maps_pending ? 1 : 0};
    key = fnv1a(key, ptrs, sizeof(ptrs));
    key = fnv1a(key, ints, sizeof(ints));
    if (rebuild_maps && !(c->params.map_cell > 0.f)) {
      const float cells[2] = {c->maps[MLOAM_MAP_SURF].auto_cell_pick(c->pinned, MLOAM_MAP_SURF),
                              c->maps[MLOAM_MAP_CORNER].auto_cell_pick(c->pinned, MLOAM_MAP_CORNER)};
      key = fnv1a(key, cells, sizeof(cells));
    }
    key = fnv1a(key, &c->params, sizeof(c->params));
    key = fnv1a(key, c->ext, sizeof(c->ext));
    key = fnv1a(key, &c->n_lidars, sizeof(c->n_lidars));
    key = fnv1a(key, &c->lidar_merge, sizeof(c->lidar_merge));
    key = fnv1a(key, c->lidar_ext, sizeof(double) * 7 * (size_t)c->n_lidars);
    key = fnv1a(key, &c->stream, sizeof(c->stream));
    {
      const void *key_now = c->cloud_key ? c->cloud_key : static_cast<const void *>(d_cloud);
      const bool have = frame_has_prefetched(c, key_now, n, n_scans);
      const bool ahead = c->next.set && c->use_lookahead;
      const int la[8] = {have ? 1 : 0, have ? c->prefetched.parity : c->frame_parity, ahead ? 1 : 0, ahead ? c->next.n : 0, ahead ? c->next.n_scans : 0,
                         (ahead && c->next.host) ? 1 : 0, (ahead && c->next_pending) ? 1 : 0, c->stamp_on ? 1 : 0};
      const void *lp[5] = {key_now, ahead ? c->next.key_ptr : nullptr, ahead ? static_cast<const void *>(c->next.d_cloud) : nullptr,
                           ahead ? static_cast<const void *>(c->next.d_scan_start) : nullptr, ahead ? static_cast<const void *>(c->next.d_scan_end) : nullptr};
      key = fnv1a(key, la, sizeof(la));
      key = fnv1a(key, lp, sizeof(lp));
    }
    Ctx::GraphEntry *e = nullptr;
    for (auto &g : c->graphs)
      if (g.key == key) e = &g;
    if (e && e->exec && e->epoch == alloc_epoch()) {
      double *stage = reinterpret_cast<double *>(c->pinned);
      for (int k = 0; k < 7; k++) stage[k] = pose_init7[k];
      if (c->has_ext)
        for (int k = 0; k < 7; k++) stage[32 + k] = c->ext[k];
      MLOAM_CUDA_OK(c, cudaGraphLaunch(e->exec, c->stream));
      c->launches += e->launches;
      c->s2m_ran = e->s2m_ran;
      c->frame_parity = (frame_has_prefetched(c, c->cloud_key ? c->cloud_key : static_cast<const void *>(d_cloud), n, n_scans) ? c->prefetched.parity : c->frame_parity) ^ 1;
      c->prefetched = e->prefetched_out;
      c->next.set = false;
      return scan2map_finish(c, e->S, pose_init7, pose_out7, stats);
    }
    if (e && e->seen >= 1) {
      if (e->exec) cudaGraphExecDestroy(e->exec), e->exec = nullptr;
      const long long l0 = c->launches;
      const unsigned long long ep0 = alloc_epoch();
      cudaGraph_t graph = nullptr;
      const Ctx::Features pf0 = c->prefetched;
      const Ctx::NextSweep nx0 = c->next;
      const int par0 = c->frame_parity;
      MLOAM_CUDA_OK(c, cudaStreamBeginCapture(c->stream, cudaStreamCaptureModeThreadLocal));
      int rc = frame_enqueue(c, d_cloud, n, d_scan_start, d_scan_end, n_scans, d_surf_map, n_surf_map, d_corner_map, n_corner_map,
                             rebuild_maps, pose_init7, &S);
      cudaError_t ce = cudaStreamEndCapture(c->stream, &graph);
      if (rc == MLOAM_OK && ce == cudaSuccess && graph && ep0 == alloc_epoch() &&
          cudaGraphInstantiate(&e->exec, graph, 0) == cudaSuccess) {
        e->launches = (int)(c->launches - l0), e->epoch = ep0, e->S = S, e->s2m_ran = c->s2m_ran;
        e->prefetched_out = c->prefetched;
        c->launches = l0;
        cudaGraphDestroy(graph);
        MLOAM_CUDA_OK(c, cudaGraphLaunch(e->exec, c->stream));
        c->launches += e->launches;
        return scan2map_finish(c, S, pose_init7, pose_out7, stats);
      }
      if (graph) cudaGraphDestroy(graph);
      cudaGetLastError();
      e->exec = nullptr, e->seen = 0;
      c->launches = l0;
      c->graph_capture_failures++;
      c->prefetched = pf0, c->next = nx0, c->frame_parity = par0;
    } else if (!e) {
      if (c->graphs.size() >= 96) {
        if (c->graphs.front().exec) cudaGraphExecDestroy(c->graphs.front().exec);
        c->graphs.erase(c->graphs.begin());
      }
      Ctx::GraphEntry g;
      g.key = key, g.seen = 1;
      c->graphs.push_back(g);
    }
  }
  int rc = frame_enqueue(c, d_cloud, n, d_scan_start, d_scan_end, n_scans, d_surf_map, n_surf_map, d_corner_map, n_corner_map,
                         rebuild_maps, pose_init7, &S);
  if (rc) return rc;
  return scan2map_finish(c, S, pose_init7, pose_out7, stats);
}

}

extern "C" {

int mloam_scan2map_device(mloam_ctx_t *h, const mloam_point_t *d_surf_scan, int n_surf, const mloam_point_t *d_corner_scan,
                          int n_corner, const double *pose_init7, double *pose_out7, mloam_solve_stats_t *stats) {
  if (!h || !pose_init7 || !pose_out7 || n_surf < 0 || n_corner < 0) return MLOAM_E_INVALID;
  cudaSetDevice(h->c.device);
  ScanRef S{reinterpret_cast<const float4 *>(d_surf_scan), n_surf, nullptr, reinterpret_cast<const float4 *>(d_corner_scan), n_corner,
            nullptr};
  return scan2map_run(&h->c, S, pose_init7, pose_out7, stats);
}

int mloam_scan2map(mloam_ctx_t *h, const mloam_point_t *h_surf_scan, int n_surf, const mloam_point_t *h_corner_scan, int n_corner,
                   const double *pose_init7, double *pose_out7, mloam_solve_stats_t *stats) {
  if (!h || !pose_init7 || !pose_out7 || n_surf < 0 || n_corner < 0) return MLOAM_E_INVALID;
  Ctx *c = &h->c;
  cudaSetDevice(c->device);
  MLOAM_CUDA_OK(c, c->scan_pts[0].reserve(sizeof(float4) * (size_t)(n_corner + 1)));
  MLOAM_CUDA_OK(c, c->scan_pts[1].reserve(sizeof(float4) * (size_t)(n_surf + 1)));
  if (n_corner > 0)
    MLOAM_CUDA_OK(c, cudaMemcpyAsync(c->scan_pts[0].p, h_corner_scan, sizeof(float4) * (size_t)n_corner, cudaMemcpyHostToDevice, c->stream));
  if (n_surf > 0)
    MLOAM_CUDA_OK(c, cudaMemcpyAsync(c->scan_pts[1].p, h_surf_scan, sizeof(float4) * (size_t)n_surf, cudaMemcpyHostToDevice, c->stream));
  ScanRef S{c->scan_pts[1].as<float4>(), n_surf, nullptr, c->scan_pts[0].as<float4>(), n_corner, nullptr};
  return scan2map_run(c, S, pose_init7, pose_out7, stats);
}

int mloam_scan2map_ua(mloam_ctx_t *h, const mloam_point_t *h_surf_scan, int n_surf, const float *h_surf_cov6,
                      const mloam_point_t *h_corner_scan, int n_corner, const float *h_corner_cov6, const double *pose_init7,
                      double *pose_out7, mloam_solve_stats_t *stats) {
  if (!h || !pose_init7 || !pose_out7 || n_surf < 0 || n_corner < 0 || (n_surf > 0 && (!h_surf_scan || !h_surf_cov6)) ||
      (n_corner > 0 && (!h_corner_scan || !h_corner_cov6)))
    return MLOAM_E_INVALID;
  Ctx *c = &h->c;
  cudaSetDevice(c->device);
  cudaStream_t st = c->stream;
  const int ns[2] = {n_corner, n_surf};
  const mloam_point_t *hp[2] = {h_corner_scan, h_surf_scan};
  const float *hc[2] = {h_corner_cov6, h_surf_cov6};
  DevBuf *cov[2] = {&c->scratch[1], &c->scratch[2]}, *sin[2] = {&c->scratch[3], &c->scratch[4]};
  for (int t = 0; t < 2; t++) {
    MLOAM_CUDA_OK(c, c->scan_pts[t].reserve(sizeof(float4) * (size_t)(ns[t] + 1)));
    MLOAM_CUDA_OK(c, cov[t]->reserve(sizeof(float) * 6 * (size_t)(ns[t] + 1)));
    MLOAM_CUDA_OK(c, sin[t]->reserve(sizeof(double) * (size_t)(ns[t] + 1)));
    if (ns[t] > 0) {
      MLOAM_CUDA_OK(c, cudaMemcpyAsync(c->scan_pts[t].p, hp[t], sizeof(float4) * (size_t)ns[t], cudaMemcpyHostToDevice, st));
      MLOAM_CUDA_OK(c, cudaMemcpyAsync(cov[t]->p, hc[t], sizeof(float) * 6 * (size_t)ns[t], cudaMemcpyHostToDevice, st));
      int rc = sqrt_info_device(c, cov[t]->as<float>(), ns[t], sin[t]->as<double>());
      if (rc) return rc;
    }
  }
  ScanRef S{c->scan_pts[1].as<float4>(), n_surf, nullptr, c->scan_pts[0].as<float4>(), n_corner, nullptr, sin[1]->as<double>(),
            sin[0]->as<double>()};
  return scan2map_run(c, S, pose_init7, pose_out7, stats);
}

int mloam_extract_features(mloam_ctx_t *h, const mloam_point_t *h_cloud, int n, const int *h_scan_start, const int *h_scan_end,
                           int n_scans, mloam_features_t *out) {
  if (!h || !out || n < 0 || n_scans <= 0 || n_scans > MLOAM_MAX_RINGS || (n > 0 && !h_cloud) || !h_scan_start || !h_scan_end)
    return MLOAM_E_INVALID;
  Ctx *c = &h->c;
  cudaSetDevice(c->device);
  out->n_sharp = out->n_less_sharp = out->n_flat = out->n_less_flat = 0;
  if (n == 0) return MLOAM_OK;
  c->prefetched.valid = false;
  FrameBufs F;
  int rc = frame_bufs(c, n, &F);
  if (rc) return rc;
  DevBuf &in = c->scratch[0];
  MLOAM_CUDA_OK(c, in.reserve(sizeof(float4) * (size_t)n + 1024 + 8 * (size_t)n_scans));
  float4 *d_cloud = in.as<float4>();
  int *d_ss = reinterpret_cast<int *>(in.as<char>() + sizeof(float4) * (size_t)n + 256);
  int *d_se = d_ss + n_scans;
  cudaStream_t st = c->stream;
  MLOAM_CUDA_OK(c, cudaMemcpyAsync(d_cloud, h_cloud, sizeof(float4) * (size_t)n, cudaMemcpyHostToDevice, st));
  MLOAM_CUDA_OK(c, cudaMemcpyAsync(d_ss, h_scan_start, sizeof(int) * n_scans, cudaMemcpyHostToDevice, st));
  MLOAM_CUDA_OK(c, cudaMemcpyAsync(d_se, h_scan_end, sizeof(int) * n_scans, cudaMemcpyHostToDevice, st));
  rc = extract_device(c, d_cloud, n, d_ss, d_se, n_scans, F.ex, nullptr, nullptr);
  if (rc) return rc;
  int *hc = reinterpret_cast<int *>(reinterpret_cast<char *>(c->pinned) + 3072);
  MLOAM_CUDA_OK(c, cudaMemcpyAsync(hc, F.ex.counts, 4 * sizeof(int), cudaMemcpyDeviceToHost, st));
  MLOAM_CUDA_OK(c, cudaMemcpyAsync(hc + 4, c->d_extract_status, sizeof(int), cudaMemcpyDeviceToHost, st));
  MLOAM_CUDA_OK(c, cudaStreamSynchronize(st));
  if (hc[4] != 0)
    return fail(c, MLOAM_E_INVALID, "extract: a ring exceeds the on-chip window (12288 points) or ScanInfo is out of range");
  if (hc[0] > out->cap || hc[1] > out->cap || hc[2] > out->cap || hc[3] > out->cap)
    return fail(c, MLOAM_E_INVALID, "extract: output capacity too small");
  out->n_sharp = hc[0], out->n_less_sharp = hc[1], out->n_flat = hc[2], out->n_less_flat = hc[3];
  if (out->corner_points_sharp && hc[0])
    MLOAM_CUDA_OK(c, cudaMemcpyAsync(out->corner_points_sharp, F.ex.sharp, sizeof(float4) * hc[0], cudaMemcpyDeviceToHost, st));
  if (out->corner_points_less_sharp && hc[1])
    MLOAM_CUDA_OK(c, cudaMemcpyAsync(out->corner_points_less_sharp, F.ex.less_sharp, sizeof(float4) * hc[1], cudaMemcpyDeviceToHost, st));
  if (out->surf_points_flat && hc[2])
    MLOAM_CUDA_OK(c, cudaMemcpyAsync(out->surf_points_flat, F.ex.flat, sizeof(float4) * hc[2], cudaMemcpyDeviceToHost, st));
  if (out->surf_points_less_flat && hc[3])
    MLOAM_CUDA_OK(c, cudaMemcpyAsync(out->surf_points_less_flat, F.ex.less_flat, sizeof(float4) * hc[3], cudaMemcpyDeviceToHost, st));
  MLOAM_CUDA_OK(c, cudaStreamSynchronize(st));
  return MLOAM_OK;
}

int mloam_extract_debug(mloam_ctx_t *h, float *h_curvature, int *h_label, int n) {
  if (!h || n < 0) return MLOAM_E_INVALID;
  Ctx *c = &h->c;
  cudaSetDevice(c->device);
  const size_t blk = (4 * ((size_t)n + 16) + 255) & ~(size_t)255;
  if (c->scratch[4].cap < 2 * blk) return fail(c, MLOAM_E_STATE, "extract_debug: no extraction of this size has run");
  const char *p = c->scratch[4].as<char>();
  if (h_curvature) MLOAM_CUDA_OK(c, cudaMemcpyAsync(h_curvature, p, sizeof(float) * n, cudaMemcpyDeviceToHost, c->stream));
  if (h_label) MLOAM_CUDA_OK(c, cudaMemcpyAsync(h_label, p + blk, sizeof(int) * n, cudaMemcpyDeviceToHost, c->stream));
  MLOAM_CUDA_OK(c, cudaStreamSynchronize(c->stream));
  return MLOAM_OK;
}

int mloam_project_cloud(mloam_ctx_t *h, const mloam_point_t *h_cloud, int n, int vertical_scans, int horizon_scans, double roi_range,
                        mloam_point_t *h_out, int *n_out, int *h_scan_start, int *h_scan_end) {
  if (!h || n < 0 || !n_out || !h_scan_start || !h_scan_end || (n > 0 && (!h_cloud || !h_out))) return MLOAM_E_INVALID;
  Ctx *c = &h->c;
  cudaSetDevice(c->device);
  *n_out = 0;
  if (vertical_scans != 16 && vertical_scans != 32 && vertical_scans != 64)
    return fail(c, MLOAM_E_INVALID, "project_cloud: vertical_scans must be 16, 32 or 64 (ImageSegmenter::setParameter)");
  if (horizon_scans <= 0) return MLOAM_E_INVALID;
  if (n == 0) {
    for (int i = 0; i < vertical_scans; i++) h_scan_start[i] = 5, h_scan_end[i] = -6;
    return MLOAM_OK;
  }
  DevBuf &in = c->scratch[0], &outb = c->scratch[1];
  MLOAM_CUDA_OK(c, in.reserve(sizeof(float4) * (size_t)n));
  MLOAM_CUDA_OK(c, outb.reserve(sizeof(float4) * (size_t)n + 1024));
  cudaStream_t st = c->stream;
  MLOAM_CUDA_OK(c, cudaMemcpyAsync(in.p, h_cloud, sizeof(float4) * (size_t)n, cudaMemcpyHostToDevice, st));
  int *d_meta = reinterpret_cast<int *>(outb.as<char>() + sizeof(float4) * (size_t)n);
  int rc = project_cloud_device(c, in.as<float4>(), n, vertical_scans, horizon_scans, roi_range, outb.as<float4>(), d_meta + 64, d_meta + 128,
                                d_meta);
  if (rc) return rc;
  int *hc = reinterpret_cast<int *>(reinterpret_cast<char *>(c->pinned) + 3072);
  MLOAM_CUDA_OK(c, cudaMemcpyAsync(hc, d_meta, sizeof(int) * 192, cudaMemcpyDeviceToHost, st));
  MLOAM_CUDA_OK(c, cudaStreamSynchronize(st));
  *n_out = hc[0];
  std::memcpy(h_scan_start, hc + 64, sizeof(int) * vertical_scans), std::memcpy(h_scan_end, hc + 128, sizeof(int) * vertical_scans);
  if (hc[0] > 0) MLOAM_CUDA_OK(c, cudaMemcpyAsync(h_out, outb.p, sizeof(float4) * (size_t)hc[0], cudaMemcpyDeviceToHost, st));
  MLOAM_CUDA_OK(c, cudaStreamSynchronize(st));
  return MLOAM_OK;
}

int mloam_voxel_downsample(mloam_ctx_t *h, const mloam_point_t *h_in, int n, float leaf, int intensity_last, mloam_point_t *h_out,
                           int *n_out) {
  if (!h || n < 0 || !n_out || (n > 0 && (!h_in || !h_out)) || !(leaf > 0.f)) return MLOAM_E_INVALID;
  Ctx *c = &h->c;
  cudaSetDevice(c->device);
  *n_out = 0;
  if (n == 0) return MLOAM_OK;
  DevBuf &in = c->scratch[0], &outb = c->scratch[1];
  MLOAM_CUDA_OK(c, in.reserve(sizeof(float4) * (size_t)n));
  MLOAM_CUDA_OK(c, outb.reserve(sizeof(float4) * (size_t)n + 256));
  cudaStream_t st = c->stream;
  MLOAM_CUDA_OK(c, cudaMemcpyAsync(in.p, h_in, sizeof(float4) * (size_t)n, cudaMemcpyHostToDevice, st));
  int *d_cnt = reinterpret_cast<int *>(outb.as<char>() + sizeof(float4) * (size_t)n);
  int rc = voxel_downsample_device(c, in.as<float4>(), n, nullptr, leaf, intensity_last, outb.as<float4>(), d_cnt, 5);
  if (rc) return rc;
  int *hc = reinterpret_cast<int *>(reinterpret_cast<char *>(c->pinned) + 3072);
  MLOAM_CUDA_OK(c, cudaMemcpyAsync(hc, d_cnt, sizeof(int), cudaMemcpyDeviceToHost, st));
  MLOAM_CUDA_OK(c, cudaStreamSynchronize(st));
  *n_out = hc[0];
  if (hc[0] > 0) MLOAM_CUDA_OK(c, cudaMemcpyAsync(h_out, outb.p, sizeof(float4) * (size_t)hc[0], cudaMemcpyDeviceToHost, st));
  MLOAM_CUDA_OK(c, cudaStreamSynchronize(st));
  return MLOAM_OK;
}

int mloam_frame_device(mloam_ctx_t *h, const mloam_point_t *d_cloud, int n, const int *d_scan_start, const int *d_scan_end, int n_scans,
                       const mloam_point_t *d_surf_map, int n_surf_map, const mloam_point_t *d_corner_map, int n_corner_map,
                       int rebuild_maps, const double *pose_init7, double *pose_out7, mloam_solve_stats_t *stats) {
  if (!h || !pose_init7 || !pose_out7 || n <= 0 || !d_cloud || !d_scan_start || !d_scan_end) return MLOAM_E_INVALID;
  cudaSetDevice(h->c.device);
  Ctx *c = &h->c;
  int rc = stage_next_sweep(c);
  if (rc) return rc;
  rc = frame_run(c, reinterpret_cast<const float4 *>(d_cloud), n, d_scan_start, d_scan_end, n_scans,
                 reinterpret_cast<const float4 *>(d_surf_map), n_surf_map, reinterpret_cast<const float4 *>(d_corner_map),
                 n_corner_map, rebuild_maps, pose_init7, pose_out7, stats);
  c->next_pending = false, c->next.set = false;
  return rc;
}

int mloam_frame_set_next_device(mloam_ctx_t *h, const mloam_point_t *d_cloud, int n, const int *d_scan_start, const int *d_scan_end, int n_scans) {
  if (!h) return MLOAM_E_INVALID;
  Ctx *c = &h->c;
  c->next = Ctx::NextSweep{};
  if (!d_cloud || n <= 0) return MLOAM_OK;
  if (!d_scan_start || !d_scan_end || n_scans <= 0 || n_scans > MLOAM_MAX_RINGS) return MLOAM_E_INVALID;
  c->next.set = true, c->next.host = false, c->next.key_ptr = d_cloud, c->next.d_cloud = reinterpret_cast<const float4 *>(d_cloud);
  c->next.d_scan_start = d_scan_start, c->next.d_scan_end = d_scan_end, c->next.n = n, c->next.n_scans = n_scans;
  return MLOAM_OK;
}
int mloam_frame_set_next(mloam_ctx_t *h, const mloam_point_t *h_cloud, int n, const int *h_scan_start, const int *h_scan_end, int n_scans) {
  if (!h) return MLOAM_E_INVALID;
  Ctx *c = &h->c;
  c->next = Ctx::NextSweep{};
  if (!h_cloud || n <= 0) return MLOAM_OK;
  if (!h_scan_start || !h_scan_end || n_scans <= 0 || n_scans > MLOAM_MAX_RINGS) return MLOAM_E_INVALID;
  c->next.set = true, c->next.host = true, c->next.key_ptr = h_cloud, c->next.n = n, c->next.n_scans = n_scans;
  c->next_host_ss = h_scan_start, c->next_host_se = h_scan_end;
  return MLOAM_OK;
}

int mloam_frame(mloam_ctx_t *h, const mloam_point_t *h_cloud, int n, const int *h_scan_start, const int *h_scan_end, int n_scans,
                const mloam_point_t *h_surf_map, int n_surf_map, const mloam_point_t *h_corner_map, int n_corner_map, int rebuild_maps,
                const double *pose_init7, double *pose_out7, mloam_solve_stats_t *stats) {
  if (!h || !pose_init7 || !pose_out7 || n <= 0 || !h_cloud || !h_scan_start || !h_scan_end || n_scans <= 0 || n_scans > MLOAM_MAX_RINGS)
    return MLOAM_E_INVALID;
  Ctx *c = &h->c;
  cudaSetDevice(c->device);
  cudaStream_t st = c->stream;
  DevBuf &in = c->scratch[0];
  MLOAM_CUDA_OK(c, in.reserve(sizeof(float4) * (size_t)n + 1024 + 8 * (size_t)n_scans));
  float4 *d_cloud = in.as<float4>();
  int *d_ss = reinterpret_cast<int *>(in.as<char>() + sizeof(float4) * (size_t)n + 256);
  int *d_se = d_ss + n_scans;
  const bool have = c->prefetched.host && frame_has_prefetched(c, h_cloud, n, n_scans);
  if (!have) {
    int *pin = reinterpret_cast<int *>(reinterpret_cast<char *>(c->pinned) + kPinnedScanInfo);
    std::memcpy(pin, h_scan_start, sizeof(int) * n_scans), std::memcpy(pin + MLOAM_MAX_RINGS, h_scan_end, sizeof(int) * n_scans);
    MLOAM_CUDA_OK(c, cudaMemcpyAsync(d_ss, pin, sizeof(int) * n_scans, cudaMemcpyHostToDevice, st));
    MLOAM_CUDA_OK(c, cudaMemcpyAsync(d_se, pin + MLOAM_MAX_RINGS, sizeof(int) * n_scans, cudaMemcpyHostToDevice, st));
    MLOAM_CUDA_OK(c, cudaMemcpyAsync(d_cloud, h_cloud, sizeof(float4) * (size_t)n, cudaMemcpyHostToDevice, st));
  }
  {
    const int rc_next = stage_next_sweep(c);
    if (rc_next) return rc_next;
  }
  const float4 *d_sm = nullptr, *d_cm = nullptr;
  if (rebuild_maps) {
    if (!h_surf_map || !h_corner_map || n_surf_map < 0 || n_corner_map < 0) return MLOAM_E_INVALID;
    DevBuf &ms = c->scratch[1], &mc = c->scratch[2];
    MLOAM_CUDA_OK(c, ms.reserve(sizeof(float4) * (size_t)(n_surf_map + 1)));
    MLOAM_CUDA_OK(c, mc.reserve(sizeof(float4) * (size_t)(n_corner_map + 1)));
    MLOAM_CUDA_OK(c, cudaMemcpyAsync(ms.p, h_surf_map, sizeof(float4) * (size_t)n_surf_map, cudaMemcpyHostToDevice, c->stream2));
    MLOAM_CUDA_OK(c, cudaMemcpyAsync(mc.p, h_corner_map, sizeof(float4) * (size_t)n_corner_map, cudaMemcpyHostToDevice, c->stream2));
    MLOAM_CUDA_OK(c, cudaEventRecord(c->ev_maps, c->stream2));
    c->maps_pending = true;
    d_sm = ms.as<float4>(), d_cm = mc.as<float4>();
  }
  c->cloud_key = h_cloud;
  const int rc = frame_run(c, d_cloud, n, d_ss, d_se, n_scans, d_sm, n_surf_map, d_cm, n_corner_map, rebuild_maps, pose_init7, pose_out7, stats);
  c->cloud_key = nullptr;
  c->maps_pending = false, c->next_pending = false, c->next.set = false;
  return rc;
}

int mloam_set_lidars(mloam_ctx_t *h, int n_lidars, const double *ext7) {
  if (!h || n_lidars < 1 || n_lidars > MLOAM_MAX_LIDARS || (n_lidars > 1 && !ext7)) return MLOAM_E_INVALID;
  Ctx *c = &h->c;
  c->n_lidars = n_lidars;
  c->prefetched.valid = false;
  c->lidar_merge = ext7 != nullptr;
  for (int l = 0; l < n_lidars; l++)
    for (int k = 0; k < 7; k++) c->lidar_ext[l][k] = ext7 ? ext7[7 * l + k] : (k == 6 ? 1.0 : 0.0);
  return MLOAM_OK;
}

int mloam_set_extrinsic(mloam_ctx_t *h, const double *ext7) {
  if (!h) return MLOAM_E_INVALID;
  Ctx *c = &h->c;
  c->has_ext = ext7 != nullptr;
  c->prefetched.valid = false;
  for (int k = 0; k < 7; k++) c->ext[k] = ext7 ? ext7[k] : (k == 6 ? 1.0 : 0.0);
  return MLOAM_OK;
}

}
```

### m-loam_b200/csrc/solve_kernels.cu

```cuda
#include "ctx.h"
#include "factors.cuh"
#include "match_fit.cuh"

namespace mloam {

constexpr int NE_H = 21, NE_G = 6;
constexpr int NE_PACK = 30;
constexpr int LIN_THREADS = 256;
constexpr int LM_THREADS = 256;

struct FeatSetDev {
  const float4 *pts;
  const unsigned char *valid;
  const float *coeff;
  int n;
  int is_plane;
  const int *d_n;
  const double *sinfo;
  const unsigned char *mask;
};
struct LinArgs {
  FeatSetDev set[2];
  int n_sets;
  double sqrt_info, huber_a;
  const double *pose;
  const LMState *state;
  int use_state;
  int respect_done;
  int lm_mode;
  int want_eig;
  double eig_thre;
  unsigned *ticket;
  LMState *state_rw;
  const P2PView *p2p;
  int two_pass;
  FitSet fit[2];
  float fit_min_plane_dis;
  int fit_check_fov;
};

__device__ __noinline__ void lm_tail(const double *partials, int n_blocks, LMState *gst, int mode, double eig_thre, int want_eig, double *out_ne,
                                     const P2PView *p2p);

template <int KFIT>
__global__ void __launch_bounds__(LIN_THREADS) k_linearize(LinArgs a, double *__restrict__ partials) {
  __shared__ double sm[LIN_THREADS / 32][NE_PACK];
  __shared__ bool is_last;
  __shared__ int barrier_failed;
  if (a.respect_done && a.state && a.state->done) {
    if (a.lm_mode != 0 && blockIdx.x == 0 && threadIdx.x == 0) a.state_rw->work[0] = 0, a.state_rw->work[1] = 0;
    return;
  }
  volatile unsigned *const gen = a.ticket + 1;
  const unsigned gen0 = a.two_pass ? *gen : 0u;
#pragma unroll 1
  for (int pass = 0; pass < (a.two_pass ? 2 : 1); pass++) {
  double xs[7];
  if (pass == 0) {
    const double *px = a.use_state == 1 ? a.state->x : (a.use_state == 2 ? a.state->xc : a.pose);
#pragma unroll
    for (int k = 0; k < 7; k++) xs[k] = px[k];
  } else {
    if (threadIdx.x == 0) {
      barrier_failed = 0;
      const long long w0 = clock64();
      while (*gen == gen0) {
        if (clock64() - w0 > 4000000000ll) {
          barrier_failed = 1;
          break;
        }
      }
      __threadfence();
    }
    __syncthreads();
    if (barrier_failed) {
      if (threadIdx.x == 0) a.state_rw->termination = 8, a.state_rw->done = 1;
      return;
    }
    if (__ldcg(&a.state_rw->done)) return;
#pragma unroll
    for (int k = 0; k < 7; k++) xs[k] = __ldcg(&a.state_rw->xc[k]);
  }
  const PoseR P = make_poser(xs);
  double acc[NE_PACK];
#pragma unroll
  for (int k = 0; k < NE_PACK; k++) acc[k] = 0.0;
  for (int s = 0; s < a.n_sets; s++) {
    const FeatSetDev fs = a.set[s];
    const int fn = fs.d_n ? min(fs.n, *fs.d_n) : fs.n;
    const int G = gridDim.x * blockDim.x, gid = blockIdx.x * blockDim.x + threadIdx.x;
    for (int i = (s & 1) ? G - 1 - gid : gid; i < fn; i += G) {
      if (KFIT > 0 && pass == 0 && a.fit[s].pos) {
        const PoseD T = pose_from_param(xs);
        fit_one<(KFIT > 0 ? KFIT : 5)>(a.fit[s], i, T, a.fit_min_plane_dis, a.fit_check_fov);
      }
      if (!fs.valid[i] || (fs.mask && !fs.mask[i])) continue;
      const float4 pf = __ldg(fs.pts + i);
      const D3 p{(double)pf.x, (double)pf.y, (double)pf.z};
      const float *cf = fs.coeff + (size_t)i * 6;
      double J[6];
      double r;
      if (fs.is_plane == 2) {
        double r3[3], J3[18];
        edge_vector_factor(P, p, D3{(double)cf[0], (double)cf[1], (double)cf[2]}, D3{(double)cf[3], (double)cf[4], (double)cf[5]}, r3,
                           J3, true);
        double rho, rho1;
        huber(a.huber_a, r3[0] * r3[0] + r3[1] * r3[1] + r3[2] * r3[2], &rho, &rho1);
        const double sc = sqrt(rho1);
#pragma unroll
        for (int m = 0; m < 3; m++) {
          const double rm = sc * r3[m];
          double Jm[6];
#pragma unroll
          for (int k = 0; k < 6; k++) Jm[k] = sc * J3[m * 6 + k];
          int q = 0;
#pragma unroll
          for (int i0 = 0; i0 < 6; i0++)
#pragma unroll
            for (int j0 = i0; j0 < 6; j0++) acc[q++] += Jm[i0] * Jm[j0];
#pragma unroll
          for (int k = 0; k < 6; k++) acc[NE_H + k] += Jm[k] * rm;
        }
        acc[NE_H + NE_G] += 0.5 * rho;
        if (s == 0) acc[NE_H + NE_G + 1] += 1.0;
        else acc[NE_H + NE_G + 2] += 1.0;
        continue;
      }
      const double si = fs.sinfo ? fs.sinfo[i] : a.sqrt_info;
      if (fs.is_plane) {
        r = plane_factor(P, p, D3{(double)cf[0], (double)cf[1], (double)cf[2]}, (double)cf[3], si, J, true);
      } else {
        r = edge_factor(P, p, D3{(double)cf[0], (double)cf[1], (double)cf[2]}, D3{(double)cf[3], (double)cf[4], (double)cf[5]},
                        si, J, true);
      }
      double rho, rho1;
      huber(a.huber_a, r * r, &rho, &rho1);
      const double sc = sqrt(rho1);
      r = sc * r;
#pragma unroll
      for (int k = 0; k < 6; k++) J[k] = sc * J[k];
      int q = 0;
#pragma unroll
      for (int i0 = 0; i0 < 6; i0++)
#pragma unroll
        for (int j0 = i0; j0 < 6; j0++) acc[q++] += J[i0] * J[j0];
#pragma unroll
      for (int k = 0; k < 6; k++) acc[NE_H + k] += J[k] * r;
      acc[NE_H + NE_G] += 0.5 * rho;
      if (s == 0) acc[NE_H + NE_G + 1] += 1.0;
      else acc[NE_H + NE_G + 2] += 1.0;
    }
  }
  const int lane = threadIdx.x & 31, wid = threadIdx.x >> 5;
  {
    double v[32];
#pragma unroll
    for (int k = 0; k < 32; k++) v[k] = k < NE_PACK ? acc[k] : 0.0;
#pragma unroll
    for (int o = 16; o > 0; o >>= 1) {
      const bool upper = (lane & o) != 0;
#pragma unroll
      for (int k = 0; k < o; k++) {
        const double send = upper ? v[k] : v[k + o];
        const double keep = upper ? v[k + o] : v[k];
        v[k] = keep + __shfl_xor_sync(MLOAM_FULL_MASK, send, o);
      }
    }
    if (lane < NE_PACK) sm[wid][lane] = v[0];
  }
  __syncthreads();
  if (threadIdx.x < NE_PACK) {
    double v = 0.0;
#pragma unroll
    for (int w = 0; w < LIN_THREADS / 32; w++) v += sm[w][threadIdx.x];
    partials[(size_t)blockIdx.x * NE_PACK + threadIdx.x] = v;
  }
  if (a.lm_mode == 0) return;
  __threadfence();
  __syncthreads();
  if (threadIdx.x == 0) is_last = atomicAdd(a.ticket, 1u) == gridDim.x - 1;
  __syncthreads();
  if (!is_last) {
    if (a.two_pass && pass == 0) continue;
    return;
  }
  __threadfence();
  lm_tail(partials, (int)gridDim.x, a.state_rw, pass == 0 ? a.lm_mode : 2, a.eig_thre, pass == 0 ? a.want_eig : 1, nullptr, a.p2p);
  __threadfence();
  __syncthreads();
  if (threadIdx.x == 0) {
    *a.ticket = 0u;
    if (a.two_pass && pass == 0) {
      __threadfence();
      atomicAdd(a.ticket + 1, 1u);
    }
  }
  }
}

__host__ __device__ void eig_sym6(const double *Ain, double *w, double *V) {
  const int N = 6;
  double a[36], v[36];
  for (int i = 0; i < 36; i++) a[i] = Ain[i], v[i] = (i % 7 == 0) ? 1.0 : 0.0;
  for (int sweep = 0; sweep < 60; sweep++) {
    double off = 0, diag = 0;
    for (int i = 0; i < N; i++) {
      diag += fabs(a[i * N + i]);
      for (int j = i + 1; j < N; j++) off += fabs(a[i * N + j]);
    }
    if (off <= 1e-22 * diag || off == 0.0) break;
    for (int p = 0; p < N - 1; p++)
      for (int q = p + 1; q < N; q++) {
        const double apq = a[p * N + q];
        if (apq == 0.0) continue;
        const double theta = (a[q * N + q] - a[p * N + p]) / (2.0 * apq);
        double t = 1.0 / (fabs(theta) + sqrt(theta * theta + 1.0));
        if (theta < 0.0) t = -t;
        const double c = 1.0 / sqrt(t * t + 1.0), s = t * c;
        a[p * N + p] -= t * apq;
        a[q * N + q] += t * apq;
        a[p * N + q] = a[q * N + p] = 0.0;
        for (int r = 0; r < N; r++) {
          if (r == p || r == q) continue;
          const double arp = a[r * N + p], arq = a[r * N + q];
          a[r * N + p] = a[p * N + r] = c * arp - s * arq;
          a[r * N + q] = a[q * N + r] = s * arp + c * arq;
        }
        for (int k = 0; k < N; k++) {
          const double vkp = v[k * N + p], vkq = v[k * N + q];
          v[k * N + p] = c * vkp - s * vkq;
          v[k * N + q] = s * vkp + c * vkq;
        }
      }
  }
  int idx[6] = {0, 1, 2, 3, 4, 5};
  for (int i = 1; i < N; i++) {
    int k = idx[i], j = i - 1;
    while (j >= 0 && a[idx[j] * N + idx[j]] > a[k * N + k]) idx[j + 1] = idx[j], j--;
    idx[j + 1] = k;
  }
  for (int j = 0; j < N; j++) {
    w[j] = a[idx[j] * N + idx[j]];
    for (int k = 0; k < N; k++) V[k * N + j] = v[k * N + idx[j]];
  }
}

void eig_report_host(const double *H36, double *w6) {
  double V[36];
  eig_sym6(H36, w6, V);
}

__device__ __forceinline__ bool chol6(double *A, double *inv_diag) {
  constexpr int N = 6;
#pragma unroll
  for (int j = 0; j < N; j++) {
    double d = A[j * N + j];
#pragma unroll
    for (int k = 0; k < j; k++) d -= A[j * N + k] * A[j * N + k];
    if (!(d > 0.0)) return false;
    d = sqrt(d);
    A[j * N + j] = d;
    const double inv = 1.0 / d;
    inv_diag[j] = inv;
#pragma unroll
    for (int i = j + 1; i < N; i++) {
      double s = A[i * N + j];
#pragma unroll
      for (int k = 0; k < j; k++) s -= A[i * N + k] * A[j * N + k];
      A[i * N + j] = s * inv;
    }
  }
  return true;
}
__device__ __forceinline__ void chol6_solve(const double *L, const double *inv_diag, const double *b, double *x) {
  constexpr int N = 6;
  double y[6];
#pragma unroll
  for (int i = 0; i < N; i++) {
    double s = b[i];
#pragma unroll
    for (int k = 0; k < i; k++) s -= L[i * N + k] * y[k];
    y[i] = s * inv_diag[i];
  }
#pragma unroll
  for (int i = N - 1; i >= 0; i--) {
    double s = y[i];
#pragma unroll
    for (int k = i + 1; k < N; k++) s -= L[k * N + i] * x[k];
    x[i] = s * inv_diag[i];
  }
}

__device__ constexpr double kMinDiag = 1e-6, kMaxDiag = 1e32, kMaxRadius = 1e16;
__device__ constexpr double kFuncTol = 1e-6, kParamTol = 1e-8, kGradTol = 1e-10, kMinRelDecrease = 1e-3;

__device__ double gradient_max_norm(const LMState *st) {
  double neg[6], xp[7];
  for (int j = 0; j < 6; j++) neg[j] = -st->g[j];
  pose_plus(st->x, neg, st->V_update, xp);
  double m = 0;
  for (int k = 0; k < 7; k++) m = fmax(m, fabs(st->x[k] - xp[k]));
  return m;
}

__device__ void lm_compute_step(LMState *st) {
  while (true) {
    if (st->iteration >= st->max_inner) {
      st->done = 1, st->termination = 0;
      return;
    }
    double Hs[36], gs[6], A[36], step[6];
#pragma unroll
    for (int a = 0; a < 6; a++) {
      gs[a] = st->scale[a] * st->g[a];
#pragma unroll
      for (int b = 0; b < 6; b++) Hs[a * 6 + b] = st->scale[a] * st->H[a * 6 + b] * st->scale[b];
    }
    if (!st->reuse_diagonal) {
#pragma unroll
      for (int j = 0; j < 6; j++) st->diag[j] = fmin(fmax(Hs[j * 6 + j], kMinDiag), kMaxDiag);
    }
#pragma unroll
    for (int i = 0; i < 36; i++) A[i] = Hs[i];
#pragma unroll
    for (int j = 0; j < 6; j++) {
      const double l = sqrt(st->diag[j] / st->radius);
      A[j * 6 + j] += l * l;
    }
    double inv_diag[6];
    bool ok = chol6(A, inv_diag);
    if (ok) {
      chol6_solve(A, inv_diag, gs, step);
#pragma unroll
      for (int j = 0; j < 6; j++) {
        step[j] = -step[j];
        if (!isfinite(step[j])) ok = false;
      }
    }
    st->reuse_diagonal = 1;
    st->iteration++;
    st->total_iterations++;
    double mcc = 0;
    if (ok) {
      double sg = 0, sHs = 0;
#pragma unroll
      for (int a = 0; a < 6; a++) {
        sg += step[a] * gs[a];
        double t = 0;
#pragma unroll
        for (int b = 0; b < 6; b++) t += Hs[a * 6 + b] * step[b];
        sHs += step[a] * t;
      }
      mcc = -(sg + 0.5 * sHs);
      if (mcc < 0) ok = false;
    }
    if (!ok) {
      if (++st->num_invalid >= 5) {
        st->done = 1, st->termination = 4;
        return;
      }
      st->radius *= 0.5;
      st->reuse_diagonal = 1;
      continue;
    }
    st->num_invalid = 0;
    double delta[6];
#pragma unroll
    for (int j = 0; j < 6; j++) delta[j] = step[j] * st->scale[j];
    pose_plus(st->x, delta, st->V_update, st->xc);
    st->model_cost_change = mcc;
    return;
  }
}

__device__ void unpack_ne(const double *ne, double *H, double *g) {
  int q = 0;
  for (int i = 0; i < 6; i++)
    for (int j = i; j < 6; j++) {
      H[i * 6 + j] = ne[q];
      H[j * 6 + i] = ne[q];
      q++;
    }
  for (int k = 0; k < 6; k++) g[k] = ne[NE_H + k];
}

__device__ void lm_advance(LMState *st, const double *ne, int mode, double eig_thre, int want_eig) {
  double H[36], g[6];
  unpack_ne(ne, H, g);
  const double cost = ne[NE_H + NE_G];
  if (mode == 1) {
    for (int i = 0; i < 36; i++) st->H[i] = H[i], st->H0[i] = H[i];
    for (int i = 0; i < 6; i++) st->g[i] = g[i];
    st->cost = cost;
    st->initial_cost = cost;
    st->n_valid[0] = (int)ne[NE_H + NE_G + 1];
    st->n_valid[1] = (int)ne[NE_H + NE_G + 2];
    st->rows = st->n_valid[0] + st->n_valid[1];
    st->skipped = 0;
    if (st->rows < st->min_corr) {
      st->done = 1, st->termination = 5, st->skipped = 1;
      for (int k = 0; k < 7; k++) st->xc[k] = st->x[k];
      return;
    }
    for (int i = 0; i < 36; i++) st->V_update[i] = (i % 7 == 0) ? 1.0 : 0.0;
    st->is_degenerate = 0;
    for (int i = 0; i < 6; i++) st->eig[i] = 0.0;
    bool need_eig = st->rows > 0 && eig_thre > 0.0;
    if (need_eig && !want_eig) {
      double S[36];
      for (int i = 0; i < 36; i++) S[i] = H[i] - ((i % 7 == 0) ? eig_thre : 0.0);
      double inv_diag[6];
      if (chol6(S, inv_diag)) need_eig = false;
    }
    if (need_eig) {
      double w[6], Vf[36], Vp[36];
      eig_sym6(H, w, Vf);
      for (int i = 0; i < 36; i++) Vp[i] = Vf[i];
      for (int j = 0; j < 6; j++) {
        if (w[j] < eig_thre) {
          for (int k = 0; k < 6; k++) Vp[k * 6 + j] = 0.0;
          st->is_degenerate = 1;
        } else {
          break;
        }
      }
      for (int i = 0; i < 6; i++) st->eig[i] = w[i];
      if (st->is_degenerate)
        for (int i = 0; i < 6; i++)
          for (int j = 0; j < 6; j++) {
            double s = 0;
            for (int k = 0; k < 6; k++) s += Vf[i * 6 + k] * Vp[j * 6 + k];
            st->V_update[i * 6 + j] = s;
          }
    }
    double xn = 0;
    for (int k = 0; k < 7; k++) xn += st->x[k] * st->x[k];
    st->x_norm = sqrt(xn);
    for (int j = 0; j < 6; j++) st->scale[j] = 1.0 / (1.0 + sqrt(H[j * 6 + j]));
    st->radius = 1e4, st->decrease_factor = 2.0, st->reuse_diagonal = 0;
    st->iteration = 0, st->num_invalid = 0, st->done = 0, st->termination = 0;
    for (int k = 0; k < 7; k++) st->xc[k] = st->x[k];
    if (gradient_max_norm(st) <= kGradTol) {
      st->done = 1, st->termination = 3;
      return;
    }
    lm_compute_step(st);
    return;
  }
  if (st->done) return;
  double sn = 0;
  for (int k = 0; k < 7; k++) sn += (st->x[k] - st->xc[k]) * (st->x[k] - st->xc[k]);
  sn = sqrt(sn);
  if (sn <= kParamTol * (st->x_norm + kParamTol)) {
    st->done = 1, st->termination = 2;
    return;
  }
  const double cost_change = st->cost - cost;
  if (fabs(cost_change) <= kFuncTol * st->cost) {
    st->done = 1, st->termination = 1;
    return;
  }
  const double rel = cost_change / st->model_cost_change;
  if (rel > kMinRelDecrease) {
    const double t = 2.0 * rel - 1.0;
    st->radius = st->radius / fmax(1.0 / 3.0, 1.0 - t * t * t);
    st->radius = fmin(kMaxRadius, st->radius);
    st->decrease_factor = 2.0;
    st->reuse_diagonal = 0;
    double xn = 0;
    for (int k = 0; k < 7; k++) st->x[k] = st->xc[k], xn += st->xc[k] * st->xc[k];
    st->x_norm = sqrt(xn);
    for (int i = 0; i < 36; i++) st->H[i] = H[i];
    for (int i = 0; i < 6; i++) st->g[i] = g[i];
    st->cost = cost;
    if (gradient_max_norm(st) <= kGradTol) {
      st->done = 1, st->termination = 3;
      return;
    }
  } else {
    st->radius = st->radius / st->decrease_factor;
    st->decrease_factor *= 2.0;
    st->reuse_diagonal = 1;
  }
  lm_compute_step(st);
}

__device__ __noinline__ void lm_tail(const double *partials, int n_blocks, LMState *gst, int mode, double eig_thre, int want_eig, double *out_ne,
                                     const P2PView *p2p) {
  __shared__ double ne[NE_PACK];
  __shared__ unsigned long long p2p_epoch;
  __shared__ int p2p_timeout;
  __shared__ double wsum[LM_THREADS / 32][32];
  __shared__ LMState s;
  static_assert(sizeof(LMState) % 8 == 0, "LMState is staged as 8-byte words");
  constexpr int kWords = (int)(sizeof(LMState) / 8);
  const long long t0 = clock64();
  if (mode != 0) {
    const unsigned long long *src = reinterpret_cast<const unsigned long long *>(gst);
    unsigned long long *dst = reinterpret_cast<unsigned long long *>(&s);
    for (int k = threadIdx.x; k < kWords; k += LM_THREADS) dst[k] = __ldcg(src + k);
  }
  {
    const int lane = threadIdx.x & 31, w = threadIdx.x >> 5;
    constexpr int S = LM_THREADS / 32;
    double v = 0.0;
    if (lane < NE_PACK) {
      const double *p = partials + lane;
      int b = w;
      for (; b + 7 * S < n_blocks; b += 8 * S) {
        double t[8];
#pragma unroll
        for (int u = 0; u < 8; u++) t[u] = __ldcg(p + (size_t)(b + u * S) * NE_PACK);
#pragma unroll
        for (int u = 0; u < 8; u++) v += t[u];
      }
      for (; b < n_blocks; b += S) v += __ldcg(p + (size_t)b * NE_PACK);
    }
    wsum[w][lane] = v;
    __syncthreads();
    if (threadIdx.x < NE_PACK) {
      double t = 0.0;
#pragma unroll
      for (int ww = 0; ww < S; ww++) t += wsum[ww][threadIdx.x];
      ne[threadIdx.x] = t;
      if (out_ne) out_ne[threadIdx.x] = t;
    }
  }
  __syncthreads();
  if (mode == 0) return;
  if (p2p) {
    const int N = p2p->nranks, me = p2p->rank;
    if (threadIdx.x == 0) p2p_epoch = *p2p->epoch, p2p_timeout = 0;
    __syncthreads();
    const unsigned long long ep = p2p_epoch;
    const int par = (int)(ep & 1ull);
    const unsigned target = (unsigned)(ep + 1ull);
    if (threadIdx.x < NE_PACK)
      for (int q = 0; q < N; q++) reinterpret_cast<volatile double *>(p2p->slots[q])[(par * MLOAM_P2P_MAX_RANKS + me) * 32 + threadIdx.x] = ne[threadIdx.x];
    __threadfence_system();
    __syncthreads();
    if (threadIdx.x < N) {
      *reinterpret_cast<volatile unsigned *>(p2p->flags[threadIdx.x] + par * MLOAM_P2P_MAX_RANKS + me) = target;
      volatile unsigned *mine = reinterpret_cast<volatile unsigned *>(p2p->flags[me] + par * MLOAM_P2P_MAX_RANKS + threadIdx.x);
      const long long w0 = clock64();
      while (true) {
        const unsigned v = *mine;
        if (v == target) break;
        if ((int)(v - target) > 0) {
          p2p_timeout = 2;
          break;
        }
        if (clock64() - w0 > 6000000000ll) {
          p2p_timeout = 1;
          break;
        }
      }
    }
    __threadfence_system();
    __syncthreads();
    if (threadIdx.x < NE_PACK) {
      double t = 0.0;
      for (int q = 0; q < N; q++) t += reinterpret_cast<volatile double *>(p2p->slots[me])[(par * MLOAM_P2P_MAX_RANKS + q) * 32 + threadIdx.x];
      ne[threadIdx.x] = t;
    }
    if (threadIdx.x == 0) *p2p->epoch = ep + 1ull;
    __syncthreads();
  }
  if (threadIdx.x == 0) {
    s.work[0] = 0, s.work[1] = 0;
    const long long t1 = clock64();
    lm_advance(&s, ne, mode, eig_thre, want_eig);
    if (p2p && p2p_timeout) s.done = 1, s.termination = 9;
    s.dbg_cycles[0] += t1 - t0, s.dbg_cycles[1] += clock64() - t1, s.dbg_cycles[2] += 1;
  }
  __syncthreads();
  {
    const unsigned long long *src = reinterpret_cast<const unsigned long long *>(&s);
    unsigned long long *dst = reinterpret_cast<unsigned long long *>(gst);
    for (int k = threadIdx.x; k < kWords; k += LM_THREADS) dst[k] = src[k];
  }
}

__global__ void __launch_bounds__(LM_THREADS) k_lm(const double *__restrict__ partials, int n_blocks, LMState *st, int mode, double eig_thre,
                                                  int want_eig, double *__restrict__ out_ne) {
  lm_tail(partials, n_blocks, st, mode, eig_thre, want_eig, out_ne, nullptr);
}

__global__ void k_lm_init(LMState *st, const double *pose7, int max_inner, int min_corr) {
  if (threadIdx.x == 0 && blockIdx.x == 0) {
    for (int k = 0; k < 7; k++) st->x[k] = pose7[k], st->xc[k] = pose7[k];
    st->max_inner = max_inner;
    st->min_corr = min_corr, st->skipped = 0;
    st->done = 0, st->termination = 0, st->total_iterations = 0, st->iteration = 0;
    st->is_degenerate = 0, st->rows = 0, st->n_valid[0] = st->n_valid[1] = 0;
    st->work[0] = st->work[1] = 0;
    st->cost = 0, st->initial_cost = 0;
    for (int i = 0; i < 36; i++) st->V_update[i] = (i % 7 == 0) ? 1.0 : 0.0, st->H0[i] = 0, st->H[i] = 0;
    for (int i = 0; i < 6; i++) st->eig[i] = 0, st->g[i] = 0;
    for (int i = 0; i < 4; i++) st->dbg_cycles[i] = 0;
  }
}

int lm_init_state(Ctx *c, const double *pose7_host, int max_inner, double eig_thre) {
  (void)eig_thre;
  MLOAM_CUDA_OK(c, c->lm_state.reserve(sizeof(LMState) + 64));
  double *stage = reinterpret_cast<double *>(c->pinned);
  for (int k = 0; k < 7; k++) stage[k] = pose7_host[k];
  double *d_stage = c->scratch[7].as<double>();
  MLOAM_CUDA_OK(c, cudaMemcpyAsync(d_stage, stage, 7 * sizeof(double), cudaMemcpyHostToDevice, c->stream));
  k_lm_init<<<1, 32, 0, c->stream>>>(c->lm_state.as<LMState>(), d_stage, max_inner, c->lm_min_corr);
  c->launches++;
  MLOAM_CUDA_OK(c, cudaGetLastError());
  return MLOAM_OK;
}

int linearize_device(Ctx *c, const FeatSet *sets, int n_sets, double sqrt_info, double huber_a, const double *d_pose7,
                     int use_state, int lm_mode, double *d_out30) {
  LinArgs a;
  int n_total = 0;
  for (int s = 0; s < 2; s++) {
    if (s < n_sets) {
      a.set[s].pts = sets[s].pts, a.set[s].valid = sets[s].valid, a.set[s].coeff = sets[s].coeff;
      a.set[s].n = sets[s].n, a.set[s].is_plane = sets[s].is_plane, a.set[s].d_n = sets[s].d_n;
      a.set[s].sinfo = sets[s].sinfo, a.set[s].mask = sets[s].mask;
      n_total = sets[s].n > n_total ? sets[s].n : n_total;
    } else {
      a.set[s].pts = nullptr, a.set[s].valid = nullptr, a.set[s].coeff = nullptr, a.set[s].n = 0, a.set[s].is_plane = 0, a.set[s].d_n = nullptr;
      a.set[s].sinfo = nullptr, a.set[s].mask = nullptr;
    }
  }
  const int want_eig = c->want_eig;
  a.n_sets = n_sets, a.sqrt_info = sqrt_info, a.huber_a = huber_a, a.pose = d_pose7;
  a.state = c->lm_state.as<LMState>();
  a.use_state = use_state;
  a.respect_done = (lm_mode == 2) ? 1 : 0;
  int nb = (n_total + LIN_THREADS - 1) / LIN_THREADS;
  if (nb < 1) nb = 1;
  const int max_nb = c->sm_count;
  if (nb > max_nb) nb = max_nb;
  if (nb > 64) nb = 64;
  MLOAM_CUDA_OK(c, c->partials.reserve(sizeof(double) * NE_PACK * (size_t)(max_nb + 3)));
  unsigned *ticket = reinterpret_cast<unsigned *>(c->partials.as<double>() + (size_t)NE_PACK * (max_nb + 2));
  if (c->ticket_zeroed_for != c->partials.p) {
    MLOAM_CUDA_OK(c, cudaMemsetAsync(ticket, 0, sizeof(double), c->stream));
    c->ticket_zeroed_for = c->partials.p;
  }
  const double eig_thre = c->lm_eig_thre >= 0.0 ? c->lm_eig_thre : c->params.eig_thre;
  const bool collective = c->nccl_comm && c->p2p_collective;
  const bool fused = lm_mode != 0 && (!collective || c->p2p_on) && !d_out30;
  a.p2p = (fused && c->p2p_on && c->p2p_collective) ? static_cast<const P2PView *>(c->p2p_view) : nullptr;
  a.lm_mode = fused ? lm_mode : 0, a.want_eig = want_eig, a.eig_thre = eig_thre, a.ticket = ticket;
  a.state_rw = c->lm_state.as<LMState>();
  a.two_pass = (c->lin_two_pass && fused && lm_mode == 1) ? 1 : 0;
  c->lin_two_pass = a.two_pass != 0;
  int kfit = 0;
  memset(a.fit, 0, sizeof(a.fit));
  a.fit_min_plane_dis = 0.f, a.fit_check_fov = 0;
  if (c->pending_fit.K) {
    if (lm_mode != 1 || n_sets != 2 || (c->pending_fit.K != 5 && c->pending_fit.K != 10)) {
      c->err = "linearize: a deferred fit is pending but this is not the first evaluation of a solve";
      c->pending_fit.K = 0;
      return MLOAM_E_STATE;
    }
    kfit = c->pending_fit.K;
    a.fit[0] = c->pending_fit.set[0], a.fit[1] = c->pending_fit.set[1];
    a.fit_min_plane_dis = c->pending_fit.min_plane_dis, a.fit_check_fov = c->pending_fit.check_fov;
    c->pending_fit.K = 0;
  }
  {
    ProfScope ps(c, "linearize");
    if (kfit == 5) k_linearize<5><<<nb, LIN_THREADS, 0, c->stream>>>(a, c->partials.as<double>());
    else if (kfit == 10) k_linearize<10><<<nb, LIN_THREADS, 0, c->stream>>>(a, c->partials.as<double>());
    else k_linearize<0><<<nb, LIN_THREADS, 0, c->stream>>>(a, c->partials.as<double>());
    c->launches++;
  }
  if (fused) {
    MLOAM_CUDA_OK(c, cudaGetLastError());
    return MLOAM_OK;
  }
  if (collective && lm_mode != 0) {
    double *ne = c->partials.as<double>() + (size_t)NE_PACK * max_nb;
    {
      ProfScope ps(c, "lm");
      k_lm<<<1, LM_THREADS, 0, c->stream>>>(c->partials.as<double>(), nb, c->lm_state.as<LMState>(), 0, 0.0, 0, ne);
      c->launches++;
    }
    int rc = comm_allreduce_doubles(c, ne, NE_PACK);
    if (rc) return rc;
    ProfScope ps(c, "lm");
    k_lm<<<1, LM_THREADS, 0, c->stream>>>(ne, 1, c->lm_state.as<LMState>(), lm_mode, (c->lm_eig_thre >= 0.0 ? c->lm_eig_thre : c->params.eig_thre), want_eig, d_out30);
    c->launches++;
  } else {
    ProfScope ps(c, "lm");
    k_lm<<<1, LM_THREADS, 0, c->stream>>>(c->partials.as<double>(), nb, c->lm_state.as<LMState>(), lm_mode, (c->lm_eig_thre >= 0.0 ? c->lm_eig_thre : c->params.eig_thre), want_eig,
                                  d_out30);
    c->launches++;
  }
  MLOAM_CUDA_OK(c, cudaGetLastError());
  return MLOAM_OK;
}

__global__ void k_factor_evaluate(int kind, int n, const double *__restrict__ points, const double *__restrict__ coeffs,
                                  const double *__restrict__ sqrt_info, const double *__restrict__ params,
                                  double *__restrict__ res, double *__restrict__ jac) {
  const int i = blockIdx.x * blockDim.x + threadIdx.x;
  if (i >= n) return;
  const D3 p{points[i * 3], points[i * 3 + 1], points[i * 3 + 2]};
  const double *cf = coeffs + (size_t)i * 6;
  const double s = sqrt_info ? sqrt_info[i] : 1.0;
  const D3 c0{cf[0], cf[1], cf[2]}, c1{cf[3], cf[4], cf[5]};
  if (kind <= 1) {
    const PoseR P = make_poser(params);
    double J[6];
    const double r = kind == 0 ? plane_factor(P, p, c0, cf[3], s, J, jac != nullptr) : edge_factor(P, p, c0, c1, s, J, jac != nullptr);
    res[i] = r;
    if (jac) {
      for (int k = 0; k < 6; k++) jac[(size_t)i * 7 + k] = J[k];
      jac[(size_t)i * 7 + 6] = 0.0;
    }
  } else if (kind == 2) {
    const PoseR P = make_poser(params);
    double r[3], J[18];
    edge_vector_factor(P, p, c0, c1, r, J, jac != nullptr);
    for (int k = 0; k < 3; k++) res[(size_t)i * 3 + k] = r[k];
    if (jac)
      for (int a = 0; a < 3; a++) {
        for (int k = 0; k < 6; k++) jac[(size_t)i * 21 + a * 7 + k] = J[a * 6 + k];
        jac[(size_t)i * 21 + a * 7 + 6] = 0.0;
      }
  } else {
    const Chain c = make_chain(params, params + 7, params + 14);
    double Jp[6], Ji[6], Je[6];
    const bool wj = jac != nullptr;
    const double r = kind == 3 ? odom_plane_factor(c, p, c0, cf[3], s, wj ? Jp : nullptr, wj ? Ji : nullptr, wj ? Je : nullptr)
                               : odom_edge_factor(c, p, c0, c1, s, wj ? Jp : nullptr, wj ? Ji : nullptr, wj ? Je : nullptr);
    res[i] = r;
    if (jac) {
      double *o = jac + (size_t)i * 21;
      for (int k = 0; k < 6; k++) o[k] = Jp[k], o[7 + k] = Ji[k], o[14 + k] = Je[k];
      o[6] = o[13] = o[20] = 0.0;
    }
  }
}

int factor_evaluate_device(Ctx *c, int kind, int n, const double *d_points, const double *d_coeffs, const double *d_sqrt_info,
                           const double *d_params, double *d_res, double *d_jac) {
  if (kind < 0 || kind > 4) {
    c->err = "factor_evaluate: kind must be 0..4";
    return MLOAM_E_INVALID;
  }
  if (n <= 0) return MLOAM_OK;
  k_factor_evaluate<<<(n + 127) / 128, 128, 0, c->stream>>>(kind, n, d_points, d_coeffs, d_sqrt_info, d_params, d_res, d_jac);
  c->launches++;
  MLOAM_CUDA_OK(c, cudaGetLastError());
  return MLOAM_OK;
}

}
```

Measured before the change: 1413.

## Speculatively run next outer-iteration KNN match on a side stream

```diff
diff --git a/m-loam_b200/csrc/api.cu b/m-loam_b200/csrc/api.cu
--- a/m-loam_b200/csrc/api.cu
+++ b/m-loam_b200/csrc/api.cu
@@ -109,13 +109,18 @@
       cudaEventCreateWithFlags(&c->ev_join5, cudaEventDisableTiming) != cudaSuccess ||
       cudaEventCreateWithFlags(&c->ev_next, cudaEventDisableTiming) != cudaSuccess ||
       cudaMallocHost(&c->pinned, kPinnedBytes) != cudaSuccess || c->lm_state.reserve(sizeof(LMState) + 64) != cudaSuccess ||
-      c->scratch[7].reserve(4096) != cudaSuccess) {
+      c->scratch[7].reserve(4096) != cudaSuccess || c->spec_slot.reserve(sizeof(SpecSlot)) != cudaSuccess) {
     delete h;
     return MLOAM_E_CUDA;
   }
   c->pinned_cap = kPinnedBytes;
   memset(c->pinned, 0, kPinnedBytes);
   cudaMemset(c->scratch[7].p, 0, 4096);
+  cudaMemset(c->spec_slot.p, 0, sizeof(SpecSlot));
+  {
+    int least = 0, greatest = 0;
+    if (cudaDeviceGetStreamPriorityRange(&least, &greatest) == cudaSuccess) c->prio_high = greatest;
+  }
   if (const char *e = getenv("MLOAM_DISABLE_GRAPHS")) c->use_graphs = (e[0] == '0' || e[0] == '\0') ? 1 : 0;
   if (const char *e = getenv("MLOAM_KNN_TRACE")) c->knn_trace_on = e[0] == '1';
   if (const char *e = getenv("MLOAM_KNN_MB")) {
@@ -148,7 +153,7 @@
   for (int i = 0; i < 4; i++) c->scan_pts[i].release(), c->feat_valid[i].release(), c->feat_coeff[i].release(), c->feat_nn[i].release(), c->knn_pos[i].release(), c->knn_changed[i].release(), c->knn_anchor[i].release(), c->knn_heavy[i].release();
   for (int i = 0; i < 2; i++) c->gf_work[i].release();
   c->knn_heavy_list.release(), c->knn_trace.release();
-  c->partials.release(), c->lm_state.release();
+  c->partials.release(), c->lm_state.release(), c->spec_slot.release();
   for (auto &s : c->scratch) s.release();
   c->frame_main.release(), c->frame_alt.release(), c->next_in.release(), c->stamps.release();
   if (c->pinned) cudaFreeHost(c->pinned);
@@ -206,6 +211,11 @@
   if (!strcmp(name, "graph_capture_failures")) {
     if (ms_total) *ms_total = 0.0;
     if (launches) *launches = c->graph_capture_failures;
+    return MLOAM_OK;
+  }
+  if (!strcmp(name, "spec_hits") || !strcmp(name, "spec_misses")) {
+    if (ms_total) *ms_total = 0.0;
+    if (launches) *launches = name[5] == 'h' ? c->spec_hits : c->spec_misses;
     return MLOAM_OK;
   }
   if (!strncmp(name, "knn_slow_rec", 12) && name[12] >= '0' && name[12] <= '9') {
@@ -248,6 +258,7 @@
   prof_collect(&h->c);
   cudaMemset(h->c.scratch[7].as<char>() + kKnnPathStatsOffset, 0, 256);
   h->c.prof.clear();
+  h->c.spec_hits = h->c.spec_misses = 0;
   return MLOAM_OK;
 }
 
diff --git a/m-loam_b200/csrc/common.cuh b/m-loam_b200/csrc/common.cuh
--- a/m-loam_b200/csrc/common.cuh
+++ b/m-loam_b200/csrc/common.cuh
@@ -169,6 +169,14 @@
   int min_corr;
   int skipped;
   long long dbg_cycles[4];
+  int spec_hits;
+  int spec_misses;
+};
+
+struct SpecSlot {
+  double pose[7];
+  int cur;
+  int pad;
 };
 
 }
diff --git a/m-loam_b200/csrc/ctx.h b/m-loam_b200/csrc/ctx.h
--- a/m-loam_b200/csrc/ctx.h
+++ b/m-loam_b200/csrc/ctx.h
@@ -25,6 +25,7 @@
   int *nn;
   int is_plane;
   const unsigned char *changed;
+  int half;
 };
 struct PendingFit {
   FitSet set[2];
@@ -215,6 +216,12 @@
   double lm_eig_thre = -1.0;
   int fuse_iter = 1;
   PendingFit pending_fit;
+  DevBuf spec_slot;
+  SpecSlot *lin_spec = nullptr;
+  bool lin_spec_count = false;
+  bool lin_priority = false;
+  int prio_high = 0;
+  long long spec_hits = 0, spec_misses = 0;
   bool lin_two_pass = false;
   int want_eig = 1;
   bool lidar_merge = false;
@@ -267,7 +274,7 @@
   int seeded;
 };
 int match_pair_device(Ctx *c, const MatchJob *jobs, int n_jobs, const double *d_pose7, const MatchCfg &cfg, int *d_work, int buf_base = 0,
-                      bool defer_fit = false);
+                      bool defer_fit = false, const SpecSlot *spec = nullptr);
 
 int match_from_scan_device(Ctx *c, int slot, int type, const float4 *d_pts, int n, const double *d_pose7, unsigned char *d_valid,
                            float *d_coeff, int *d_nn3);
@@ -287,7 +294,7 @@
 };
 int linearize_device(Ctx *c, const FeatSet *sets, int n_sets, double sqrt_info, double huber_a, const double *d_pose7,
                      int use_state, int lm_mode, double *d_out29);
-int lm_init_state(Ctx *c, const double *pose7_host, int max_inner, double eig_thre);
+int lm_init_state(Ctx *c, const double *pose7_host, int max_inner, double eig_thre, SpecSlot *spec = nullptr);
 void eig_report_host(const double *H36, double *w6);
 int factor_evaluate_device(Ctx *c, int kind, int n, const double *d_points, const double *d_coeffs, const double *d_sqrt_info,
                            const double *d_params, double *d_res, double *d_jac);
diff --git a/m-loam_b200/csrc/match_kernels.cu b/m-loam_b200/csrc/match_kernels.cu
--- a/m-loam_b200/csrc/match_kernels.cu
+++ b/m-loam_b200/csrc/match_kernels.cu
@@ -18,6 +18,7 @@
   int seeded;
   unsigned char *changed;
   float4 *anchor;
+  int half;
   const unsigned char *heavy_in;
   unsigned char *heavy_out;
 };
@@ -33,7 +34,7 @@
 template <int K, int MB>
 __global__ void __launch_bounds__(MWARPS * 32, MB)
     k_match_knn(KnnSet a, KnnSet b, const double *__restrict__ pose7, float min_match_sq_dis, HeavyQ hq,
-                unsigned *__restrict__ path_stats, unsigned tma_min, unsigned *__restrict__ trace) {
+                unsigned *__restrict__ path_stats, unsigned tma_min, unsigned *__restrict__ trace, const int *__restrict__ cur) {
   __shared__ KnnSmem ksm[MWARPS];
   const int lane = threadIdx.x & 31;
   KnnSmem &ks = ksm[threadIdx.x >> 5];
@@ -42,7 +43,20 @@
   knn_smem_init(ks, lane, tma_min);
   __shared__ GridP s_grid[2];
   __shared__ PoseD s_pose;
-  if (threadIdx.x == 0) s_grid[0] = load_grid(a.map), s_grid[1] = load_grid(b.map), s_pose = pose_from_param(pose7);
+  __shared__ int *s_pos[2][2];
+  __shared__ float4 *s_anchor[2][2];
+  __shared__ unsigned char *s_changed[2];
+  if (threadIdx.x == 0) {
+    s_grid[0] = load_grid(a.map), s_grid[1] = load_grid(b.map), s_pose = pose_from_param(pose7);
+    const int h = cur ? (*cur & 1) : 0;
+    const KnnSet *sets[2] = {&a, &b};
+    for (int t = 0; t < 2; t++) {
+      const size_t in = (size_t)sets[t]->half * (size_t)h, out = (size_t)sets[t]->half * (size_t)(h ^ 1);
+      s_pos[t][0] = sets[t]->pos + in * K, s_pos[t][1] = sets[t]->pos + out * K;
+      s_anchor[t][0] = sets[t]->anchor + in, s_anchor[t][1] = sets[t]->anchor + out;
+      s_changed[t] = sets[t]->changed ? sets[t]->changed + out : nullptr;
+    }
+  }
   __syncthreads();
   const int na = a.d_n ? min(a.n, *a.d_n) : a.n;
   const int nb = b.d_n ? min(b.n, *b.d_n) : b.n;
@@ -73,19 +87,18 @@
     const float3 sel = associate(s_pose, p.x, p.y, p.z);
     const GridP &g = s_grid[in_a ? 0 : 1];
     Best best;
-    int *const pos_out = (in_a ? a.pos : b.pos) + (size_t)j * K;
     const int seeded = in_a ? a.seeded : b.seeded;
-    unsigned char *const changed = in_a ? a.changed : b.changed;
-    float4 *const anchor = (in_a ? a.anchor : b.anchor) + j;
+    const int set = in_a ? 0 : 1;
     int prev = -1, newpos = -1;
     bool done = false;
     float r2 = 3.0e38f;
     if (seeded) {
-      if (lane < K) prev = pos_out[lane];
-      const float4 an = *anchor;
+      if (lane < K) prev = s_pos[set][0][(size_t)j * K + lane];
+      const float4 an = s_anchor[set][0][j];
       const float mx = sel.x - an.x, my = sel.y - an.y, mz = sel.z - an.z;
       const float moved = sqrtf(mx * mx + my * my + mz * mz);
       const bool within = an.w > 0.0f && moved + 2e-5f < an.w;
+      if (within && (in_a ? a.half : b.half) && lane == 0) s_anchor[set][1][j] = an;
       if (__shfl_sync(MLOAM_FULL_MASK, prev, 0) < 0) {
         if (within) {
           done = true;
@@ -115,7 +128,7 @@
           }
           if (!(r2 < min_match_sq_dis)) {
             newpos = -1;
-            if (lane == 0) *anchor = make_float4(sel.x, sel.y, sel.z, 0.0f);
+            if (lane == 0) s_anchor[set][1][j] = make_float4(sel.x, sel.y, sel.z, 0.0f);
           }
           done = true;
           path = 0;
@@ -167,10 +180,10 @@
         if (kK != MLOAM_KEY_NONE) lbK = fminf(lbK, sqrtf(key_d2(kK)));
         slack = lbK - sqrtf(min_match_sq_dis) - 2e-5f;
       }
-      if (lane == 0) *anchor = make_float4(sel.x, sel.y, sel.z, slack);
-    }
-    if (lane < K) pos_out[lane] = newpos;
-    if (changed) {
+      if (lane == 0) s_anchor[set][1][j] = make_float4(sel.x, sel.y, sel.z, slack);
+    }
+    if (lane < K) s_pos[set][1][(size_t)j * K + lane] = newpos;
+    if (unsigned char *const changed = s_changed[set]) {
       const bool diff = __any_sync(MLOAM_FULL_MASK, lane < K && (!seeded || newpos != prev));
       if (lane == 0) changed[j] = diff ? 1 : 0;
     }
@@ -210,7 +223,8 @@
   }
 }
 
-int match_pair_device(Ctx *c, const MatchJob *jobs, int n_jobs, const double *d_pose7, const MatchCfg &cfg, int *d_work, int buf_base, bool defer_fit) {
+int match_pair_device(Ctx *c, const MatchJob *jobs, int n_jobs, const double *d_pose7, const MatchCfg &cfg, int *d_work, int buf_base, bool defer_fit,
+                      const SpecSlot *spec) {
   (void)d_work;
   if (n_jobs < 1 || n_jobs > 2 || (buf_base != 0 && buf_base != 2)) {
     c->err = "match: 1 or 2 jobs";
@@ -240,14 +254,16 @@
       c->err = "match_from_map: type must be 'c' or 's'";
       return MLOAM_E_INVALID;
     }
+    const size_t per_copy = (size_t)(J.n + 1), copies = spec ? 2 : 1;
     DevBuf &pb = c->knn_pos[buf_base + t];
-    MLOAM_CUDA_OK(c, pb.reserve(sizeof(int) * (size_t)K * (size_t)(J.n + 1)));
+    MLOAM_CUDA_OK(c, pb.reserve(sizeof(int) * (size_t)K * per_copy * copies));
     k.map = c->maps[J.slot].view();
     DevBuf &cb = c->knn_changed[buf_base + t];
-    MLOAM_CUDA_OK(c, cb.reserve((size_t)(J.n + 1)));
+    MLOAM_CUDA_OK(c, cb.reserve(per_copy * copies));
     k.pts = J.pts, k.n = J.n, k.d_n = J.d_n, k.pos = pb.as<int>();
+    k.half = spec ? (int)per_copy : 0;
     DevBuf &ab = c->knn_anchor[buf_base + t];
-    MLOAM_CUDA_OK(c, ab.reserve(sizeof(float4) * (size_t)(J.n + 1)));
+    MLOAM_CUDA_OK(c, ab.reserve(sizeof(float4) * per_copy * copies));
     k.seeded = J.seeded, k.changed = cb.as<unsigned char>(), k.anchor = ab.as<float4>();
     DevBuf &hb = c->knn_heavy[buf_base + t];
     const size_t half = ((size_t)J.n + 256) & ~(size_t)255;
@@ -255,7 +271,8 @@
     k.heavy_in = J.seeded ? hb.as<unsigned char>() + half * (size_t)c->knn_parity : nullptr;
     k.heavy_out = hb.as<unsigned char>() + half * (size_t)(J.seeded ? (c->knn_parity ^ 1) : c->knn_parity);
     flip = flip || J.seeded;
-    f.changed = (J.seeded && !J.nn) ? cb.as<unsigned char>() : nullptr;
+    f.changed = ((J.seeded || spec) && !J.nn) ? cb.as<unsigned char>() : nullptr;
+    f.half = k.half;
     f.sorted = k.map.sorted, f.pts = J.pts, f.n = J.n, f.d_n = J.d_n, f.pos = pb.as<int>();
     f.valid = J.valid, f.coeff = J.coeff, f.nn = J.nn, f.is_plane = J.type == 's' ? 1 : 0;
     n_upper += J.n;
@@ -296,7 +313,8 @@
     int nb = (n_upper + MWARPS - 1) / MWARPS;
     if (nb > mb * c->sm_count) nb = mb * c->sm_count;
 #define MLOAM_LAUNCH_KNN(KK, MBB) \
-  k_match_knn<KK, MBB><<<nb, MWARPS * 32, 0, st>>>(ks[0], ks[1], d_pose7, cfg.min_match_sq_dis, hq, path_stats, c->knn_tma_min, trace)
+  k_match_knn<KK, MBB><<<nb, MWARPS * 32, 0, st>>>(ks[0], ks[1], d_pose7, cfg.min_match_sq_dis, hq, path_stats, c->knn_tma_min, trace, \
+                                                   spec ? &spec->cur : nullptr)
     if (K == 5) {
       if (mb == 2) MLOAM_LAUNCH_KNN(5, 2);
       else if (mb == 3) MLOAM_LAUNCH_KNN(5, 3);
diff --git a/m-loam_b200/csrc/pipeline.cu b/m-loam_b200/csrc/pipeline.cu
--- a/m-loam_b200/csrc/pipeline.cu
+++ b/m-loam_b200/csrc/pipeline.cu
@@ -26,27 +26,32 @@
   if (rc) return rc;
   rc = reserve_feat(c, 1, S.n_surf);
   if (rc) return rc;
-  rc = lm_init_state(c, pose_init7, P.max_inner, P.eig_thre);
+  const int nc_use = P.point_edge_factor ? S.n_corner : 0, ns_use = P.point_plane_factor ? S.n_surf : 0;
+  const bool spec = c->fuse_iter && P.max_inner == 1 && P.gf_method == 0 && (!c->nccl_comm || c->p2p_on) && (nc_use > 0 || ns_use > 0);
+  SpecSlot *slot = spec ? c->spec_slot.as<SpecSlot>() : nullptr;
+  rc = lm_init_state(c, pose_init7, P.max_inner, P.eig_thre, slot);
   if (rc) return rc;
   LMState *st = c->lm_state.as<LMState>();
   const double *d_pose = st->x;
   const double sinfo = map_sqrt_info(P.cov_trace);
   const MatchCfg cfg = match_cfg(c);
   int *h_done = reinterpret_cast<int *>(reinterpret_cast<char *>(c->pinned) + 2048);
-  const int nc_use = P.point_edge_factor ? S.n_corner : 0, ns_use = P.point_plane_factor ? S.n_surf : 0;
   FeatSet sets[2] = {
       FeatSet{S.corner, c->feat_valid[0].as<unsigned char>(), c->feat_coeff[0].as<float>(), nc_use, 0, S.d_n_corner, S.sinfo_corner},
       FeatSet{S.surf, c->feat_valid[1].as<unsigned char>(), c->feat_coeff[1].as<float>(), ns_use, 1, S.d_n_surf, S.sinfo_surf}};
+  auto match = [&](int outer, const double *pose) {
+    const int seeded = (outer > 0 && c->use_seeds) ? 1 : 0;
+    MatchJob jobs[2] = {
+        MatchJob{MLOAM_MAP_CORNER, 'c', S.corner, nc_use, S.d_n_corner, c->feat_valid[0].as<unsigned char>(),
+                 c->feat_coeff[0].as<float>(), nullptr, seeded},
+        MatchJob{MLOAM_MAP_SURF, 's', S.surf, ns_use, S.d_n_surf, c->feat_valid[1].as<unsigned char>(),
+                 c->feat_coeff[1].as<float>(), nullptr, seeded}};
+    const bool defer_fit = c->fuse_iter && P.gf_method == 0;
+    return match_pair_device(c, jobs, 2, pose, cfg, &st->work[0], 0, defer_fit, slot);
+  };
   for (int outer = 0; outer < P.max_outer; outer++) {
-    {
-      const int seeded = (outer > 0 && c->use_seeds) ? 1 : 0;
-      MatchJob jobs[2] = {
-          MatchJob{MLOAM_MAP_CORNER, 'c', S.corner, nc_use, S.d_n_corner, c->feat_valid[0].as<unsigned char>(),
-                   c->feat_coeff[0].as<float>(), nullptr, seeded},
-          MatchJob{MLOAM_MAP_SURF, 's', S.surf, ns_use, S.d_n_surf, c->feat_valid[1].as<unsigned char>(),
-                   c->feat_coeff[1].as<float>(), nullptr, seeded}};
-      const bool defer_fit = c->fuse_iter && P.gf_method == 0;
-      rc = match_pair_device(c, jobs, 2, d_pose, cfg, &st->work[0], 0, defer_fit);
+    if (!spec || outer == 0) {
+      rc = match(outer, d_pose);
       if (rc) return rc;
       stamp(c, "match");
     }
@@ -73,22 +78,45 @@
     }
     if (P.gf_method != 0) stamp(c, "gf");
     c->want_eig = 0;
-    c->lin_two_pass = c->fuse_iter && P.max_inner == 1;
+    c->lin_two_pass = c->fuse_iter && P.max_inner == 1 && !spec;
+    c->lin_spec = slot, c->lin_spec_count = outer > 0;
     rc = linearize_device(c, sets, 2, sinfo, P.huber_a, nullptr, 1, 1, nullptr);
     c->want_eig = 1;
+    c->lin_spec = nullptr;
     const bool second_done = c->lin_two_pass;
     c->lin_two_pass = false;
     if (rc) return rc;
-    stamp(c, second_done ? "linearize x2" : "linearize");
+    stamp(c, spec ? "linearize A (fit, x, LM step)" : second_done ? "linearize x2" : "linearize");
+    const bool fork_spec = spec && outer + 1 < P.max_outer;
+    if (fork_spec && !c->prof_on) MLOAM_CUDA_OK(c, cudaEventRecord(c->ev_fork3, c->stream));
     for (int it = 0; it < P.max_inner && !second_done; it++) {
+      c->lin_priority = fork_spec;
       rc = linearize_device(c, sets, 2, sinfo, P.huber_a, nullptr, 2, 2, nullptr);
+      c->lin_priority = false;
       if (rc) return rc;
-      stamp(c, "linearize (candidate)");
+      stamp(c, spec ? "linearize B (xc, LM accept)" : "linearize (candidate)");
       if (P.max_inner > 1) {
         MLOAM_CUDA_OK(c, cudaMemcpyAsync(h_done, &st->done, sizeof(int), cudaMemcpyDeviceToHost, c->stream));
         MLOAM_CUDA_OK(c, cudaStreamSynchronize(c->stream));
         if (*h_done) break;
       }
+    }
+    if (fork_spec) {
+      const cudaStream_t main_stream = c->stream;
+      if (!c->prof_on) {
+        MLOAM_CUDA_OK(c, cudaStreamWaitEvent(c->stream3, c->ev_fork3, 0));
+        c->stream = c->stream3;
+      }
+      stamp(c, "side: (fork)");
+      rc = match(outer + 1, slot->pose);
+      stamp(c, "side: speculative match");
+      c->stream = main_stream;
+      if (rc) return rc;
+      if (!c->prof_on) {
+        MLOAM_CUDA_OK(c, cudaEventRecord(c->ev_join3, c->stream3));
+        MLOAM_CUDA_OK(c, cudaStreamWaitEvent(c->stream, c->ev_join3, 0));
+      }
+      stamp(c, "speculative match join");
     }
   }
   char *pin = reinterpret_cast<char *>(c->pinned);
@@ -117,6 +145,7 @@
     return fail(c, MLOAM_E_NCCL, "scan2map: peer-memory exchange failed (a rank did not arrive or the ranks lost lock-step); "
                                   "call mloam_comm_p2p_reset on every rank behind a barrier");
   }
+  c->spec_hits += hs->spec_hits, c->spec_misses += hs->spec_misses;
   if (hs->termination == 8) {
     for (int k = 0; k < 7; k++) pose_out7[k] = pose_init7[k];
     if (stats) stats->ran = 1, stats->termination = 8;
@@ -413,7 +442,7 @@
                              rebuild_maps, pose_init7, &S);
       cudaError_t ce = cudaStreamEndCapture(c->stream, &graph);
       if (rc == MLOAM_OK && ce == cudaSuccess && graph && ep0 == alloc_epoch() &&
-          cudaGraphInstantiate(&e->exec, graph, 0) == cudaSuccess) {
+          cudaGraphInstantiate(&e->exec, graph, cudaGraphInstantiateFlagUseNodePriority) == cudaSuccess) {
         e->launches = (int)(c->launches - l0), e->epoch = ep0, e->S = S, e->s2m_ran = c->s2m_ran;
         e->prefetched_out = c->prefetched;
         c->launches = l0;
diff --git a/m-loam_b200/csrc/solve_kernels.cu b/m-loam_b200/csrc/solve_kernels.cu
--- a/m-loam_b200/csrc/solve_kernels.cu
+++ b/m-loam_b200/csrc/solve_kernels.cu
@@ -37,6 +37,8 @@
   FitSet fit[2];
   float fit_min_plane_dis;
   int fit_check_fov;
+  SpecSlot *spec;
+  int spec_count;
 };
 
 __device__ __noinline__ void lm_tail(const double *partials, int n_blocks, LMState *gst, int mode, double eig_thre, int want_eig, double *out_ne,
@@ -47,6 +49,7 @@
   __shared__ double sm[LIN_THREADS / 32][NE_PACK];
   __shared__ bool is_last;
   __shared__ int barrier_failed;
+  __shared__ int spec_half;
   if (a.respect_done && a.state && a.state->done) {
     if (a.lm_mode != 0 && blockIdx.x == 0 && threadIdx.x == 0) a.state_rw->work[0] = 0, a.state_rw->work[1] = 0;
     return;
@@ -60,6 +63,15 @@
     const double *px = a.use_state == 1 ? a.state->x : (a.use_state == 2 ? a.state->xc : a.pose);
 #pragma unroll
     for (int k = 0; k < 7; k++) xs[k] = px[k];
+    if (KFIT > 0 && a.spec) {
+      if (threadIdx.x == 0) {
+        long long diff = 0;
+#pragma unroll
+        for (int k = 0; k < 7; k++) diff |= __double_as_longlong(xs[k]) ^ __double_as_longlong(a.spec->pose[k]);
+        spec_half = diff == 0 ? (a.spec->cur & 1) ^ 1 : -1;
+      }
+      __syncthreads();
+    }
   } else {
     if (threadIdx.x == 0) {
       barrier_failed = 0;
@@ -90,9 +102,14 @@
     const int fn = fs.d_n ? min(fs.n, *fs.d_n) : fs.n;
     const int G = gridDim.x * blockDim.x, gid = blockIdx.x * blockDim.x + threadIdx.x;
     for (int i = (s & 1) ? G - 1 - gid : gid; i < fn; i += G) {
-      if (KFIT > 0 && pass == 0 && a.fit[s].pos) {
+      if (KFIT > 0 && pass == 0 && a.fit[s].pos && !(a.spec && spec_half < 0)) {
         const PoseD T = pose_from_param(xs);
-        fit_one<(KFIT > 0 ? KFIT : 5)>(a.fit[s], i, T, a.fit_min_plane_dis, a.fit_check_fov);
+        FitSet f = a.fit[s];
+        if (a.spec) {
+          const unsigned off = (unsigned)(spec_half * f.half);
+          f.pos += off * (KFIT > 0 ? KFIT : 5), f.changed += off;
+        }
+        fit_one<(KFIT > 0 ? KFIT : 5)>(f, i, T, a.fit_min_plane_dis, a.fit_check_fov);
       }
       if (!fs.valid[i] || (fs.mask && !fs.mask[i])) continue;
       const float4 pf = __ldg(fs.pts + i);
@@ -189,6 +206,16 @@
   __threadfence();
   __syncthreads();
   if (threadIdx.x == 0) {
+    if (KFIT > 0 && a.spec) {
+      const bool hit = spec_half >= 0;
+      if (hit) a.spec->cur = spec_half;
+      if (a.spec_count) {
+        int *const n = hit ? &a.state_rw->spec_hits : &a.state_rw->spec_misses;
+        *n = __ldcg(n) + 1;
+      }
+#pragma unroll
+      for (int k = 0; k < 7; k++) a.spec->pose[k] = __ldcg(&a.state_rw->xc[k]);
+    }
     *a.ticket = 0u;
     if (a.two_pass && pass == 0) {
       __threadfence();
@@ -586,7 +613,7 @@
   lm_tail(partials, n_blocks, st, mode, eig_thre, want_eig, out_ne, nullptr);
 }
 
-__global__ void k_lm_init(LMState *st, const double *pose7, int max_inner, int min_corr) {
+__global__ void k_lm_init(LMState *st, const double *pose7, int max_inner, int min_corr, SpecSlot *spec) {
   if (threadIdx.x == 0 && blockIdx.x == 0) {
     for (int k = 0; k < 7; k++) st->x[k] = pose7[k], st->xc[k] = pose7[k];
     st->max_inner = max_inner;
@@ -598,17 +625,20 @@
     for (int i = 0; i < 36; i++) st->V_update[i] = (i % 7 == 0) ? 1.0 : 0.0, st->H0[i] = 0, st->H[i] = 0;
     for (int i = 0; i < 6; i++) st->eig[i] = 0, st->g[i] = 0;
     for (int i = 0; i < 4; i++) st->dbg_cycles[i] = 0;
-  }
-}
-
-int lm_init_state(Ctx *c, const double *pose7_host, int max_inner, double eig_thre) {
+    st->spec_hits = st->spec_misses = 0;
+    if (spec)
+      for (int k = 0; k < 7; k++) spec->pose[k] = pose7[k];
+  }
+}
+
+int lm_init_state(Ctx *c, const double *pose7_host, int max_inner, double eig_thre, SpecSlot *spec) {
   (void)eig_thre;
   MLOAM_CUDA_OK(c, c->lm_state.reserve(sizeof(LMState) + 64));
   double *stage = reinterpret_cast<double *>(c->pinned);
   for (int k = 0; k < 7; k++) stage[k] = pose7_host[k];
   double *d_stage = c->scratch[7].as<double>();
   MLOAM_CUDA_OK(c, cudaMemcpyAsync(d_stage, stage, 7 * sizeof(double), cudaMemcpyHostToDevice, c->stream));
-  k_lm_init<<<1, 32, 0, c->stream>>>(c->lm_state.as<LMState>(), d_stage, max_inner, c->lm_min_corr);
+  k_lm_init<<<1, 32, 0, c->stream>>>(c->lm_state.as<LMState>(), d_stage, max_inner, c->lm_min_corr, spec);
   c->launches++;
   MLOAM_CUDA_OK(c, cudaGetLastError());
   return MLOAM_OK;
@@ -653,6 +683,12 @@
   a.state_rw = c->lm_state.as<LMState>();
   a.two_pass = (c->lin_two_pass && fused && lm_mode == 1) ? 1 : 0;
   c->lin_two_pass = a.two_pass != 0;
+  a.spec = c->lin_spec, a.spec_count = c->lin_spec_count ? 1 : 0;
+  if (a.spec && (!fused || lm_mode != 1 || a.two_pass || !c->pending_fit.K)) {
+    c->err = "linearize: speculative re-association needs the fused tail and the deferred fit of its match";
+    c->pending_fit.K = 0;
+    return MLOAM_E_STATE;
+  }
   int kfit = 0;
   memset(a.fit, 0, sizeof(a.fit));
   a.fit_min_plane_dis = 0.f, a.fit_check_fov = 0;
@@ -671,7 +707,13 @@
     ProfScope ps(c, "linearize");
     if (kfit == 5) k_linearize<5><<<nb, LIN_THREADS, 0, c->stream>>>(a, c->partials.as<double>());
     else if (kfit == 10) k_linearize<10><<<nb, LIN_THREADS, 0, c->stream>>>(a, c->partials.as<double>());
-    else k_linearize<0><<<nb, LIN_THREADS, 0, c->stream>>>(a, c->partials.as<double>());
+    else if (c->lin_priority) {
+      cudaLaunchConfig_t lc = {};
+      cudaLaunchAttribute at[1];
+      at[0].id = cudaLaunchAttributePriority, at[0].val.priority = c->prio_high;
+      lc.gridDim = dim3(nb), lc.blockDim = dim3(LIN_THREADS), lc.dynamicSmemBytes = 0, lc.stream = c->stream, lc.attrs = at, lc.numAttrs = 1;
+      MLOAM_CUDA_OK(c, cudaLaunchKernelEx(&lc, k_linearize<0>, a, c->partials.as<double>()));
+    } else k_linearize<0><<<nb, LIN_THREADS, 0, c->stream>>>(a, c->partials.as<double>());
     c->launches++;
   }
   if (fused) {
```

Result: faster. 1521, median of 6 (+7.7%).
